# charles-kmc/Semi-blind-image-deblurring-problems-with-TV

Hardware: AMD Instinct MI355X
Metric: SALSA outer-iters/sec + final PSNR, 2048x2048 Gaussian blur (higher is better)
Workload: dtype f64; 1 GPU; SALSA_v2 TV deblur, one 2048x2048 image per GPU, Gaussian PSF 7x7, BSNR 30 dB, TViters=10; images_per_gpu=1, parallelism=images x1

## Files before the change

include/sbtv.h:

```cpp
#ifndef SBTV_H
#define SBTV_H

#include <stddef.h>

#ifdef __cplusplus
extern "C" {
#endif

#define SBTV_VERSION 100

#define SBTV_HOST_PTRS   0
#define SBTV_DEVICE_PTRS 1
#define SBTV_REDUCE_DEVICE  2
#define SBTV_SAPG_HOST_LOOP 4
#define SBTV_FISTA_EXACT_PROX 2

#define SBTV_OK                   0
#define SBTV_ERR_BADARG          -1
#define SBTV_ERR_SIZE            -2
#define SBTV_ERR_MAXITER         -3
#define SBTV_ERR_DUALVARS        -4
#define SBTV_ERR_MODE            -5
#define SBTV_ERR_STOPCRITERION   -6
#define SBTV_ERR_INIT            -7
// ... 200 lines not shown
                       int chambolleit, unsigned long long seed, int chain_offset, const double *noise,
                       double *x_out, const sbtv_moments_opts *mo, double *post_mean, double *post_var,
                       long long *post_count, int flags);

typedef struct sbtv_myula_wavelet_opts {
    int    samples;
    double lambda, gamma;
    unsigned long long seed;
    int    chain_offset;
} sbtv_myula_wavelet_opts;
int sbtv_myula_wavelet(sbtv_ctx *ctx, const double *y, int M, int N, int batch,
                       const double *taps, int taille, const double *h, int hlen, int levels,
                       const sbtv_myula_wavelet_opts *op,
                       const double *theta, const double *sigma2,
                       const double *xw0, const double *noise,
                       double *gx, double *logpi,
                       double *xw_last,
                       const sbtv_moments_opts *mo,
                       double *post_mean, double *post_var, long long *post_count,
                       double *coef_mean, double *coef_var,
                       int flags);

int sbtv_max_eigenval(sbtv_ctx *ctx, const double *taps, int taille, const double *x0,
                      int M, int N, double tol, int max_iter, double *val, int *iters, int flags);

int sbtv_PSNR(sbtv_ctx *ctx, const double *x_true, const double *x, int M, int N, int batch, double *out, int flags);
int sbtv_MSE(sbtv_ctx *ctx, const double *x_true, const double *x, int M, int N, int batch, double *out, int flags);

typedef struct sbtv_group sbtv_group;
int         sbtv_group_create(const int *devices, int n, sbtv_group **out);
int         sbtv_group_destroy(sbtv_group *g);
int         sbtv_group_size(const sbtv_group *g);
sbtv_ctx   *sbtv_group_ctx(sbtv_group *g, int i);
const char *sbtv_group_last_error(const sbtv_group *g);
int         sbtv_group_shard_of(const sbtv_group *g, int n_items, int item, int *shard, int *first, int *count);
int sbtv_SALSA_v2_sharded(sbtv_group *g, const double *y, int M, int N, int n_items,
                          const double *taps, int taille, const double *tau, const double *mu,
                          const sbtv_salsa_opts *opts, const double *true_x, const double *x_init,
                          double *x_out, double *objective, double *distance, double *times, double *mses,
                          int *numA, int *numAt, int *n_outer);
int sbtv_SALSA_v2_sharded_dev(sbtv_group *g, const double *const *y, int M, int N, int n_items,
                              const double *taps, int taille, const double *tau, const double *mu,
                              const sbtv_salsa_opts *opts, const double *const *true_x,
                              const double *const *x_init, double *const *x_out, double *objective,
                              double *distance, double *times, double *mses, int *numA, int *numAt, int *n_outer);
int sbtv_SAPG_algorithm_sharded(sbtv_group *g, const double *y, int M, int N, int n_items,
                                const sbtv_sapg_opts *op, const double *x0, const double *noise,
                                double *thetas, double *ps, double *sigmas, double *logpi,
                                double *logpi_wu, double *gx, double *grads, double *eb, double *x_last);
int sbtv_fista_tv_sharded(sbtv_group *g, const double *b, int M, int N, int n_items,
                          const double *taps, int taille, const double *tau, double L,
                          int prox_iters, int stopcriterion, double tolerance, int maxiters,
                          int zero_start, const double *true_x, double *x_out,
                          double *objective, double *mses, int *n_iter);
int sbtv_CSALSA_v2_sharded(sbtv_group *g, const double *y, int M, int N, int n_items,
                           const double *taps, int taille, const double *mu1, const double *mu2,
                           const double *sigma, const double *epsilon, double continuationfactor,
                           const sbtv_salsa_opts *opts, const double *true_x, const double *x_init,
                           double *x_out, double *objective, double *distance1, double *distance2,
                           double *criterion, double *times, double *mses,
                           int *numA, int *numAt, int *n_outer);
int sbtv_CoRAL_v2_sharded(sbtv_group *g, const double *y, int M, int N, int n_items,
                          const double *taps, int taille, const double *tau1, const double *tau2,
                          const double *mu1, const double *mu2, const double *mu_ls, int TViters2,
                          const sbtv_salsa_opts *opts, const double *true_x, const double *x_init,
                          double *x_out, double *objective, double *distance, double *times, double *mses,
                          int *numA, int *numAt, int *n_outer);
int sbtv_SALSA_masked_sharded(sbtv_group *g, const double *y, const double *mask, int M, int N, int n_items,
                              const double *taps, int taille, const double *tau, const double *mu1, const double *mu2,
                              const sbtv_salsa_opts *opts, const double *true_x, const double *x_init,
                              double *x_out, double *objective, double *distance, double *times, double *mses,
                              int *numA, int *numAt, int *n_outer);

int sbtv_host_transpose(const double *src, double *dst, int batch, int rows, int cols);
int sbtv_diag_solve_stats(const sbtv_ctx *ctx, double out[4]);
int sbtv_diag_stage_stats(const sbtv_ctx *ctx, double out[4]);
int sbtv_diag_canary(sbtv_ctx *ctx, int poke, int *enabled, int *nbuf, int *nbad);
int sbtv_last_host_stats(const sbtv_ctx *ctx, double out[14]);
int sbtv_diag_workspace(sbtv_ctx *ctx, const char *name, void **dptr, size_t *bytes);
int sbtv_diag_switches(char *buf, size_t cap);
int sbtv_diag_time_pass(sbtv_ctx *ctx, int pass, int M, int N, int batch, int reps, double *ms_avg, double *alg_bytes);
int sbtv_diag_prox_variant(sbtv_ctx *ctx, int M, int N, int batch, int out[6]);
int sbtv_diag_prox_geometry(sbtv_ctx *ctx, int M, int N, int batch, int out[16]);
int sbtv_diag_fft_plan(sbtv_ctx *ctx, int M, int N, int batch, int out[16]);
typedef struct sbtv_diag_pass {
    int M, N, batch, op, epilogue, taille, shared_spec, repeats;
    const double *x, *add;
    const double *taps, *d1taps, *d2taps;
    const double *y, *e0;
    const double *mu, *cs;
    const int *frozen;
    const double *u, *bu_in, *tru, *xprev, *sub_b;
    double alpha;
    double *bu, *ystep;
    double *x_out, *g_out, *acc, *sums, *tv;
} sbtv_diag_pass;
int sbtv_diag_spectral_pass(sbtv_ctx *ctx, const sbtv_diag_pass *args);

#ifdef __cplusplus
}
#endif
#endif
```

semi-blind-image-deblurring-problems-with-tv_amd/csrc/admm.hip:

```cpp
#include <chrono>
#include <cmath>

#include "sbtv_internal.h"

#pragma clang fp contract(off)

namespace sbtv {

namespace {

constexpr int AB = 256;

__device__ __forceinline__ double ad_wave_sum(double v) {
#pragma unroll
    for (int off = 32; off > 0; off >>= 1) v += __shfl_xor(v, off, 64);
    return v;
}

template <int NQ>
__device__ __forceinline__ void ad_store_partials(double (&acc)[NQ], double *__restrict__ partials) {
    __shared__ double red[NQ * 4];
    const int lane = threadIdx.x & 63, w = threadIdx.x >> 6;
#pragma unroll
    for (int c = 0; c < NQ; ++c) {
// ... 350 lines not shown
    double2 *S, *Hs, *Ys;
    double *taps_d;
    double inv_scale, parseval;
    bool spectral = false;
};

int admm_common(sbtv_ctx *ctx, int M, int N, const double *taps, int taille, const double *yd, AdmmCommon *c) {
    if (((size_t)M * N) & 1)
        return fail(ctx, SBTV_ERR_SIZE, "this entry point needs an even number of pixels (its element-wise passes move two per lane)");
    SBTV_TRY(fft_plan(ctx, M, N, 1, &c->fp));
    c->P = (size_t)M * N;
    SBTV_TRY(ws_get_t(ctx, "admm.S", c->fp.s_img, &c->S));
    SBTV_TRY(ws_get_t(ctx, "admm.H", c->fp.u_img, &c->Hs));
    SBTV_TRY(ws_get_t(ctx, "admm.Y", c->fp.u_img, &c->Ys));
    SBTV_TRY(ws_get_t(ctx, "admm.taps", (size_t)taille * taille, &c->taps_d));
    SBTV_HIP(ctx, hipMemcpyAsync(c->taps_d, taps, sizeof(double) * taille * taille, hipMemcpyHostToDevice, ctx->stream));
    SBTV_HIP(ctx, hipStreamSynchronize(ctx->stream));
    c->inv_scale = 1.0 / ((double)c->fp.n1 * N);
    c->parseval = 1.0 / ((double)M * N);
    SBTV_TRY(psf_spectrum(ctx, c->fp, c->taps_d, taille, c->Hs));
    if (yd) {
        RowsArgs a{};
        a.dir_fwd = 1;
        a.op = OP_NONE;
        SBTV_TRY(fft_cols_fwd(ctx, c->fp, yd, nullptr, c->S));
        SBTV_TRY(fft_rows(ctx, c->fp, c->S, c->S, a));
        SBTV_TRY(spec_unpack(ctx, c->fp, c->S, c->Ys));
    }
    return 0;
}

int admm_apply(sbtv_ctx *ctx, const AdmmCommon &c, int op, const double *in, double *out) {
    RowsArgs a{};
    a.dir_fwd = 1;
    a.dir_inv = 1;
    a.op = op;
    a.H = c.Hs;
    SBTV_TRY(fft_cols_fwd(ctx, c.fp, in, nullptr, c.S));
    SBTV_TRY(fft_rows(ctx, c.fp, c.S, c.S, a));
    return fft_cols_inv(ctx, c.fp, c.S, out, c.inv_scale);
}

int admm_init_x(sbtv_ctx *ctx, const AdmmCommon &c, int initialization, const double *yd, const double *xi, double *x) {
    if (initialization == 0) {
        SBTV_HIP(ctx, hipMemsetAsync(x, 0, sizeof(double) * c.P, ctx->stream));
    } else if (initialization == 2) {
        SBTV_TRY(admm_apply(ctx, c, OP_MUL_HC, yd, x));
    } else {
        SBTV_HIP(ctx, hipMemcpyAsync(x, xi, sizeof(double) * c.P, hipMemcpyDeviceToDevice, ctx->stream));
    }
    return 0;
}

int check_common(sbtv_ctx *ctx, const char *who, const double *y, const double *taps, const sbtv_salsa_opts *opts,
                 const double *x_init, int M, int N, int batch, int taille) {
    if (!y || !opts || batch < 1) return fail(ctx, SBTV_ERR_BADARG, std::string(who) + ": missing required argument");
    if (!taps) return fail(ctx, SBTV_ERR_MISSING_AT, "The function handle for transpose of A is missing");
    if (opts->stopcriterion < 1 || opts->stopcriterion > 3) return fail(ctx, SBTV_ERR_STOPCRITERION, "Unknown stopping criterion");
    if (opts->initialization != 0 && opts->initialization != 2 && opts->initialization != 33333)
        return fail(ctx, SBTV_ERR_INIT, "Unknown 'Initialization' option");
    if (opts->initialization == 33333 && !x_init) return fail(ctx, SBTV_ERR_INIT, "Initialization = array but x_init is NULL");
    if (opts->TViters <= 0) return fail(ctx, SBTV_ERR_MAXITER, std::string(who) + ": TViters must be positive");
    if (opts->maxiter < 1) return fail(ctx, SBTV_ERR_MAXITER, std::string(who) + ": maxiter must be positive");
    if (taille < 1 || taille > 15 || taille > M || taille > N) return fail(ctx, SBTV_ERR_PSF, "Mask does not fit inside array");
    return 0;
}

inline bool csalsa_spectral_wanted() {
    static const bool on = [] {
        const char *e = getenv("SBTV_CSALSA_SPECTRAL");
        return !(e && e[0] == '0');
    }();
    return on;
}

inline int admm_prox(sbtv_ctx *ctx, const ProxPlan &pp, const double *g, int K, double *f, bool spec, long long *nlaunch,
                     double *stepsums, const double *lam_dev, double tol, double tau) {
    if (!spec) {
        SBTV_TRY(prox_reset(ctx, pp, lam_dev, 1.0, K, tol, tau, true, nullptr));
        return prox_iterate(ctx, pp, g, K, f);
    }
    SBTV_TRY(prox_iterate(ctx, pp, g, K, f, false, 1, (int)(*nlaunch & 1), nullptr));
    *nlaunch += prox_launches(pp, K);
    return reduce_partials(ctx, pp.partials, K, pp.fnblk, stepsums);
}

struct AdmmSlots {
    hipEvent_t ev[2] = {nullptr, nullptr};
    ~AdmmSlots() {
        for (auto e : ev)
            if (e) (void)hipEventDestroy(e);
    }
};

int csalsa_one(sbtv_ctx *ctx, const double *yd, int M, int N, const double *taps, int taille, double mu1, double mu2,
               double sigma, double epsilon, double delta, const sbtv_salsa_opts *opts, const double *td,
               const double *xi, double *x_out_dev, double *objective, double *distance1, double *distance2,
               double *criterion, double *times, double *mses, int *numA, int *numAt, int *n_outer, bool spec_wanted) {
    AdmmCommon c;
    {
        FftPlan chk;
        SBTV_TRY(fft_plan(ctx, M, N, 1, &chk));
        const bool sp = delta == 1.0 && csalsa_spectral_wanted() && fft_rows_csalsa_ok(chk) && !(M & 1) &&
                        (size_t)M * N < ((size_t)1 << 31);
        SBTV_TRY(admm_common(ctx, M, N, taps, taille, sp ? yd : nullptr, &c));
        c.spectral = sp;
    }
    const bool spectral = c.spectral;
    ProxPlan pp;
    SBTV_TRY(prox_plan(ctx, M, N, 1, &pp));
    const size_t P = c.P;
    const int nb = ad_blocks(P);
    double *xbuf[2], *u, *bu, *v, *bv, *w, *Ax, *g, *par, *partials, *sums, *acc;
    double2 *Ws;
    SBTV_TRY(ws_get_t(ctx, "admm.acc", (size_t)3 * fft_rows_blocks(c.fp), &acc));
    SBTV_TRY(ws_get_t(ctx, "admm.x0", P, &xbuf[0]));
    SBTV_TRY(ws_get_t(ctx, "admm.x1", P, &xbuf[1]));
    SBTV_TRY(ws_get_t(ctx, "admm.u", P, &u));
    SBTV_TRY(ws_get_t(ctx, "admm.bu", P, &bu));
    SBTV_TRY(ws_get_t(ctx, "admm.v", P, &v));
    SBTV_TRY(ws_get_t(ctx, "admm.bv", P, &bv));
    SBTV_TRY(ws_get_t(ctx, "admm.w", P, &w));
    SBTV_TRY(ws_get_t(ctx, "admm.Ax", P, &Ax));
    SBTV_TRY(ws_get_t(ctx, "admm.g", P, &g));
    SBTV_TRY(ws_get_t(ctx, "admm.par", (size_t)4, &par));
    SBTV_TRY(ws_get_t(ctx, "admm.partials", (size_t)8 * nb, &partials));
    SBTV_TRY(ws_get_t(ctx, "admm.sums", (size_t)64, &sums));
    SBTV_TRY(ws_get_t(ctx, "admm.W", c.fp.u_img, &Ws));
    double2 *Es = Ws;
    double *cst = nullptr, *rs = nullptr;
    SBTV_TRY(ws_get_t(ctx, "admm.cs", (size_t)8, &cst));
    SBTV_TRY(ws_get_t(ctx, "admm.rs", (size_t)4, &rs));
    double *hs = nullptr;
    {
        void *pz = nullptr;
        SBTV_TRY(pinned_get(ctx, sizeof(double) * 128, &pz));
        hs = static_cast<double *>(pz);
    }
    const int maxiter = opts->maxiter;
    if (!(epsilon != 0.0)) epsilon = sqrt((double)P + 8 * sqrt((double)P)) * sigma;
    auto upload_par = [&]() -> int {
        const double h[4] = {mu1, mu2, 1.0 / mu1, 0.0};
        SBTV_HIP(ctx, hipMemcpyAsync(par, h, sizeof(h), hipMemcpyHostToDevice, ctx->stream));
        SBTV_HIP(ctx, hipStreamSynchronize(ctx->stream));
        return 0;
    };
    SBTV_TRY(upload_par());
    int h_numA = 0, h_numAt = 1;
    ctx->calls += 2;
    double *x = xbuf[0];
    SBTV_TRY(admm_init_x(ctx, c, opts->initialization, yd, xi, x));
    if (opts->initialization == 0) ctx->calls += 1;
    if (opts->initialization == 2) h_numAt += 1;
    SBTV_HIP(ctx, hipMemsetAsync(u, 0, sizeof(double) * P, ctx->stream));
    SBTV_HIP(ctx, hipMemsetAsync(bu, 0, sizeof(double) * P, ctx->stream));
    SBTV_HIP(ctx, hipMemsetAsync(v, 0, sizeof(double) * P, ctx->stream));
    SBTV_HIP(ctx, hipMemsetAsync(bv, 0, sizeof(double) * P, ctx->stream));
    SBTV_TRY(prox_zero_duals(ctx, pp));
    SBTV_TRY(prox_reset(ctx, pp, par + 2, 1.0, opts->TViters, opts->chambolle_tol, opts->chambolle_tau, false, nullptr));

    SBTV_TRY(admm_apply(ctx, c, OP_MUL_H, x, Ax));
    h_numA += 2;
    ctx->calls += 2;
    {
        double *sv, *sbv, *sbu;
        SBTV_TRY(ws_get_t(ctx, "admm.scratch0", P, &sv));
        SBTV_TRY(ws_get_t(ctx, "admm.scratch1", P, &sbv));
        SBTV_TRY(ws_get_t(ctx, "admm.scratch2", P, &sbu));
        SBTV_HIP(ctx, hipMemsetAsync(sbv, 0, sizeof(double) * P, ctx->stream));
        SBTV_HIP(ctx, hipMemsetAsync(sbu, 0, sizeof(double) * P, ctx->stream));
        SBTV_HIP(ctx, hipMemsetAsync(sums, 0, sizeof(double) * 16, ctx->stream));
        hipLaunchKernelGGL(csalsa_update_kernel, dim3(nb), dim3(AB), 0, ctx->stream, Ax, yd, x, u, sv, sbv, sbu, td,
                           (const double *)nullptr, sums + 8, 1.0, partials, P);
        SBTV_TRY(reduce_partials(ctx, partials, 6, nb, sums));
        SBTV_TRY(tvnorm_dev(ctx, x, M, N, 1, sums + 6));
        SBTV_HIP(ctx, hipMemcpyAsync(hs, sums, sizeof(double) * 8, hipMemcpyDeviceToHost, ctx->stream));
        SBTV_HIP(ctx, hipStreamSynchronize(ctx->stream));
        if (criterion) criterion[0] = sqrt(hs[0]);
        if (distance1) distance1[0] = sqrt(hs[0]);
        if (distance2) distance2[0] = sqrt(hs[2]);
        if (objective) objective[0] = hs[6];
        if (mses && td) mses[0] = hs[3] / (double)P;
        if (times) times[0] = 0.0;
    }
    double crit_prev = sqrt(hs[0]), obj_prev = hs[6];
    const auto t0 = std::chrono::steady_clock::now();
    SBTV_HIP(ctx, hipEventRecord(ctx->ev[0], ctx->stream));
    const int K = opts->TViters;
    const bool spec = spec_wanted && delta == 1.0 && prox_spec_ok(pp, g, u, K);
    const int lag = (spec && (opts->speculate & 1)) ? 1 : 0;
    long long nlaunch = 0, prox_iters = 0;
    AdmmSlots slots;
    for (auto &e : slots.ev) SBTV_HIP(ctx, hipEventCreateWithFlags(&e, hipEventDisableTiming));
    double *hslot[2] = {hs, hs + 64};
    const bool tv_fused = fft_cols_tv_ok(c.fp);
    const int ntv = tv_fused ? fft_cols_blocks(c.fp) : 0;
    double *tvp = nullptr;
    if (tv_fused) SBTV_TRY(ws_get_t(ctx, "admm.tvc", (size_t)ntv, &tvp));
    if (spectral) {
        const double h[8] = {mu2, mu2, 0.0, 0.0, 0.0, 0.0, 0.0, 0.0};
        SBTV_HIP(ctx, hipMemsetAsync(Es, 0, sizeof(double2) * c.fp.u_img, ctx->stream));
        SBTV_HIP(ctx, hipMemcpyAsync(cst, h, sizeof(h), hipMemcpyHostToDevice, ctx->stream));
        SBTV_HIP(ctx, hipStreamSynchronize(ctx->stream));
    }
    auto enqueue_spectral = [&](int outer) -> int {
        const int k = outer - 1;
        double *xn = xbuf[k & 1];
        const double *xprev = xbuf[(k & 1) ^ 1];
        RowsArgs a{};
        a.dir_fwd = 1;
        a.dir_inv = 1;
        a.op = OP_CSALSA;
        a.H = c.Hs;
        a.Y = c.Ys;
        a.E = Es;
        a.cs = cst;
        a.mu = par;
        a.acc = acc;
        SBTV_TRY(fft_cols_fwd(ctx, c.fp, u, bu, c.S));
        SBTV_TRY(fft_rows(ctx, c.fp, c.S, c.S, a));
        if (fft_cols_inv_step_ok(c.fp)) {
            SBTV_TRY(fft_cols_inv_sub(ctx, c.fp, c.S, xn, c.inv_scale, bu, g));
        } else {
            SBTV_TRY(fft_cols_inv(ctx, c.fp, c.S, xn, c.inv_scale));
            hipLaunchKernelGGL(ad_sub_kernel, dim3(nb), dim3(AB), 0, ctx->stream, xn, bu, g, P);
        }
        hipLaunchKernelGGL(csalsa_scal_kernel, dim3(1), dim3(256), 0, ctx->stream, acc, fft_rows_blocks(c.fp), cst, epsilon,
                           c.parseval, sums);
        RedJobs jb;
        if (!spec) {
            SBTV_TRY(admm_prox(ctx, pp, g, K, u, false, &nlaunch, sums + 16, par + 2, opts->chambolle_tol, opts->chambolle_tau));
        } else {
            SBTV_TRY(prox_iterate(ctx, pp, g, K, u, false, 1, (int)(nlaunch & 1), nullptr));
            nlaunch += prox_launches(pp, K);
            jb.add(pp.partials, K, pp.fnblk, sums + 16);
        }
        hipLaunchKernelGGL(csalsa_post_kernel, dim3(nb), dim3(AB), 0, ctx->stream, xn, u, bu, td,
                           (opts->stopcriterion == 2) ? xprev : (const double *)nullptr, partials, (unsigned)M, (unsigned)N, P);
        jb.add(partials, 5, nb, sums + 2);
        SBTV_TRY(reduce_jobs(ctx, jb));
        SBTV_HIP(ctx, hipGetLastError());
        double *hsl = hslot[outer & 1];
        SBTV_HIP(ctx, hipMemcpyAsync(hsl, sums, sizeof(double) * (16 + (spec ? K : 0)), hipMemcpyDeviceToHost, ctx->stream));
        if (!spec) SBTV_HIP(ctx, hipMemcpyAsync(hsl + 8, pp.ctrl, sizeof(int), hipMemcpyDeviceToHost, ctx->stream));
        SBTV_HIP(ctx, hipEventRecord(slots.ev[outer & 1], ctx->stream));
        return 0;
    };
    auto enqueue = [&](int outer) -> int {
        if (spectral) return enqueue_spectral(outer);
        const int k = outer - 1;
        double *xn = xbuf[k & 1];
        const double *xprev = xbuf[(k & 1) ^ 1];
        hipLaunchKernelGGL(csalsa_w_kernel, dim3(nb), dim3(AB), 0, ctx->stream, yd, v, bv, par, w, P);
        {
            RowsArgs a{};
            a.dir_fwd = 1;
            a.op = OP_NONE;
            SBTV_TRY(fft_cols_fwd(ctx, c.fp, w, nullptr, c.S));
            SBTV_TRY(fft_rows(ctx, c.fp, c.S, c.S, a));
            SBTV_TRY(spec_unpack(ctx, c.fp, c.S, Ws));
        }
        {
            RowsArgs a{};
            a.dir_fwd = 1;
            a.dir_inv = 1;
            a.op = OP_SALSA;
            a.H = c.Hs;
            a.Y = Ws;
            a.mu = par;
            a.acc = acc;
            SBTV_TRY(fft_cols_fwd(ctx, c.fp, u, bu, c.S));
            SBTV_TRY(fft_rows(ctx, c.fp, c.S, c.S, a));
            SBTV_TRY(fft_cols_inv(ctx, c.fp, c.S, xn, c.inv_scale));
        }
        hipLaunchKernelGGL(ad_sub_kernel, dim3(nb), dim3(AB), 0, ctx->stream, xn, bu, g, P);
        SBTV_TRY(admm_prox(ctx, pp, g, K, u, spec, &nlaunch, sums + 16, par + 2, opts->chambolle_tol, opts->chambolle_tau));
        {
            RowsArgs a{};
            a.dir_fwd = 1;
            a.dir_inv = 1;
            a.op = OP_MUL_H;
            a.H = c.Hs;
            SBTV_TRY(fft_cols_fwd_f(ctx, c.fp, xn, nullptr, c.S, nullptr, tvp));
            SBTV_TRY(fft_rows(ctx, c.fp, c.S, c.S, a));
            SBTV_TRY(fft_cols_inv(ctx, c.fp, c.S, Ax, c.inv_scale));
        }
        hipLaunchKernelGGL(csalsa_ve_kernel, dim3(nb), dim3(AB), 0, ctx->stream, Ax, yd, bv, partials, P);
        SBTV_TRY(reduce_partials(ctx, partials, 1, nb, sums + 8));
        hipLaunchKernelGGL(csalsa_update_kernel, dim3(nb), dim3(AB), 0, ctx->stream, Ax, yd, xn, u, v, bv, bu, td,
                           (opts->stopcriterion == 2) ? xprev : (const double *)nullptr, sums + 8, epsilon, partials, P);
        SBTV_TRY(reduce_partials(ctx, partials, 6, nb, sums));
        if (tv_fused) SBTV_TRY(reduce_partials(ctx, tvp, 1, ntv, sums + 6));
        else SBTV_TRY(tvnorm_dev(ctx, xn, M, N, 1, sums + 6));
        SBTV_HIP(ctx, hipGetLastError());
        double *hsl = hslot[outer & 1];
        SBTV_HIP(ctx, hipMemcpyAsync(hsl, sums, sizeof(double) * (16 + (spec ? K : 0)), hipMemcpyDeviceToHost, ctx->stream));
        if (!spec) SBTV_HIP(ctx, hipMemcpyAsync(hsl + 8, pp.ctrl, sizeof(int), hipMemcpyDeviceToHost, ctx->stream));
        SBTV_HIP(ctx, hipEventRecord(slots.ev[outer & 1], ctx->stream));
        return 0;
    };
    bool stop = false;
    auto process = [&](int outer) -> int {
        const int k = outer - 1;
        const double *hsl = hslot[outer & 1];
        SBTV_HIP(ctx, hipEventSynchronize(slots.ev[outer & 1]));
        if (spec) SBTV_TRY(spec_stop_rule(ctx, pp, hsl + 16, K, opts->chambolle_tol));
        prox_iters += spec ? K : *reinterpret_cast<const int *>(hsl + 8);
        h_numAt += 1;
        h_numA += 1;
        ctx->calls += 3;
        const double crit = sqrt(hsl[0]), obj = hsl[6];
        if (criterion) criterion[k] = crit;
        if (distance1) distance1[k] = sqrt(hsl[1]);
        if (distance2) distance2[k] = sqrt(hsl[2]);
        if (objective) objective[k] = obj;
        if (mses && td) mses[k] = hsl[3] / (double)P;
        if (times) times[k] = std::chrono::duration<double>(std::chrono::steady_clock::now() - t0).count();
        if (delta != 1.0) {
// ... 62 lines not shown
    {
        void *pz = nullptr;
        SBTV_TRY(pinned_get(ctx, sizeof(double) * 192, &pz));
        hs = static_cast<double *>(pz);
    }
    {
        const double h[4] = {mu_ls, tau1 / mu1, tau2 / mu2, 0.0};
        SBTV_HIP(ctx, hipMemcpyAsync(par, h, sizeof(h), hipMemcpyHostToDevice, ctx->stream));
        SBTV_HIP(ctx, hipStreamSynchronize(ctx->stream));
    }
    const int maxiter = opts->maxiter;
    int h_numA = 0, h_numAt = 2;
    ctx->calls += 3;
    double *x = xbuf[0];
    SBTV_TRY(admm_init_x(ctx, c, opts->initialization, yd, xi, x));
    if (opts->initialization == 0) ctx->calls += 1;
    for (double *dst : {u, bu, v, bv})
        SBTV_HIP(ctx, hipMemcpyAsync(dst, x, sizeof(double) * P, hipMemcpyDeviceToDevice, ctx->stream));
    SBTV_HIP(ctx, hipMemsetAsync(g1, 0, sizeof(double) * P, ctx->stream));
    SBTV_HIP(ctx, hipMemsetAsync(g2, 0, sizeof(double) * P, ctx->stream));
    SBTV_TRY(prox_zero_duals(ctx, pu));
    SBTV_TRY(prox_reset(ctx, pu, par + 1, 1.0, opts->TViters, opts->chambolle_tol, opts->chambolle_tau, false, nullptr));
    if (!batched) {
        SBTV_TRY(prox_zero_duals(ctx, pv));
        SBTV_TRY(prox_reset(ctx, pv, par + 2, 1.0, TViters2, opts->chambolle_tol, opts->chambolle_tau, false, nullptr));
    }

    {
        RowsArgs a{};
        a.dir_fwd = 1;
        a.op = OP_RESID;
        a.H = c.Hs;
        a.Y = c.Ys;
        a.acc = acc;
        SBTV_TRY(fft_cols_fwd(ctx, c.fp, x, nullptr, c.S));
        SBTV_TRY(fft_rows(ctx, c.fp, c.S, nullptr, a));
        SBTV_TRY(reduce_partials(ctx, acc, 1, nrb, sums + 8));
        SBTV_TRY(tvnorm_dev(ctx, u, M, N, 1, sums + 9));
        SBTV_HIP(ctx, hipMemsetAsync(sums, 0, sizeof(double) * 8, ctx->stream));
        if (td) {
            double *o4 = nullptr;
            SBTV_TRY(ws_get_t(ctx, "admm.o4", (size_t)4, &o4));
            SBTV_TRY(pair_sums(ctx, x, td, P, 1, o4));
            SBTV_HIP(ctx, hipMemcpyAsync(sums, o4, sizeof(double), hipMemcpyDeviceToDevice, ctx->stream));
        }
        SBTV_HIP(ctx, hipMemcpyAsync(hs, sums, sizeof(double) * 16, hipMemcpyDeviceToHost, ctx->stream));
        SBTV_HIP(ctx, hipStreamSynchronize(ctx->stream));
        h_numA += 1;
        ctx->calls += 1;
        const double f0 = 0.5 * (hs[8] * c.parseval) + tau1 * hs[9] + tau2 * hs[9];
        if (objective) objective[0] = f0;
        if (times) times[0] = 0.0;
        if (mses && td) mses[0] = hs[0] / (double)P;
        hs[15] = f0;
    }
    double obj_prev = hs[15];
    const auto t0 = std::chrono::steady_clock::now();
    SBTV_HIP(ctx, hipEventRecord(ctx->ev[0], ctx->stream));
    const int K1 = opts->TViters, K2 = TViters2;
    const bool spec = spec_wanted && prox_spec_ok(pu, g1, u, K1) &&
                      (batched || prox_spec_ok(pv, g2, v, K2));
    const int lag = (spec && (opts->speculate & 1)) ? 1 : 0;
    long long nl_u = 0, nl_v = 0, prox_iters = 0;
    AdmmSlots slots;
    for (auto &e : slots.ev) SBTV_HIP(ctx, hipEventCreateWithFlags(&e, hipEventDisableTiming));
    double *hslot[2] = {hs, hs + 96};
    auto enqueue = [&](int outer) -> int {
        double *xn = xbuf[outer & 1];
        const double *xprev = xbuf[(outer & 1) ^ 1];
        const bool sp = spec && outer >= 2;
        RedJobs jb;
        if (spec && outer == 2) {
            SBTV_TRY(prox_reset(ctx, pu, par + 1, 1.0, K1, opts->chambolle_tol, opts->chambolle_tau, true, nullptr));
            if (!batched) SBTV_TRY(prox_reset(ctx, pv, par + 2, 1.0, K2, opts->chambolle_tol, opts->chambolle_tau, true, nullptr));
        }
        if (batched) {
            static_assert(FSTRIDE == 32, "the step sums of the second prox are read at sums + 48");
            if (!sp) {
                SBTV_TRY(prox_reset(ctx, pu, par + 1, 1.0, K1, opts->chambolle_tol, opts->chambolle_tau, true, nullptr));
                SBTV_TRY(prox_iterate(ctx, pu, g1, K1, u));
            } else {
                SBTV_TRY(prox_iterate(ctx, pu, g1, K1, u, false, 1, (int)(nl_u & 1), nullptr));
                nl_u += prox_launches(pu, K1);
                jb.add(pu.partials, FSTRIDE + K1, pu.fnblk, sums + 16);
            }
        } else {
            SBTV_TRY(admm_prox(ctx, pu, g1, K1, u, sp, &nl_u, sums + 16, par + 1, opts->chambolle_tol, opts->chambolle_tau));
            SBTV_TRY(admm_prox(ctx, pv, g2, K2, v, sp, &nl_v, sums + 48, par + 2, opts->chambolle_tol, opts->chambolle_tau));
        }
        if (tv_in_s) {
            hipLaunchKernelGGL(coral_s_kernel<true>, dim3(nb), dim3(AB), 0, ctx->stream, u, bu, v, bv, mu1, mu2, mu_ls, s, tvpart,
                               (unsigned)M, (unsigned)N, P);
            jb.add(tvpart, 2, nb, sums + 9);
        } else {
            hipLaunchKernelGGL(coral_s_kernel<false>, dim3(nb), dim3(AB), 0, ctx->stream, u, bu, v, bv, mu1, mu2, mu_ls, s, tvpart,
                               (unsigned)M, (unsigned)N, P);
        }
        {
            RowsArgs a{};
            a.dir_fwd = 1;
            a.dir_inv = 1;
            a.op = OP_SALSA;
            a.H = c.Hs;
            a.Y = c.Ys;
            a.mu = par;
            a.acc = acc;
            SBTV_TRY(fft_cols_fwd(ctx, c.fp, s, nullptr, c.S));
            SBTV_TRY(fft_rows(ctx, c.fp, c.S, c.S, a));
            SBTV_TRY(fft_cols_inv(ctx, c.fp, c.S, xn, c.inv_scale));
        }
        hipLaunchKernelGGL(coral_post_kernel, dim3(nb), dim3(AB), 0, ctx->stream, xn,
                           (opts->stopcriterion == 2) ? xprev : (const double *)nullptr, u, v, bu, bv, g1, g2, td, partials, P);
        jb.add(partials, 7, nb, sums);
        jb.add(acc, 1, nrb, sums + 8);
        SBTV_TRY(reduce_jobs(ctx, jb));
        if (!tv_in_s) {
            SBTV_TRY(tvnorm_dev(ctx, u, M, N, 1, sums + 9));
            SBTV_TRY(tvnorm_dev(ctx, v, M, N, 1, sums + 10));
        }
        SBTV_HIP(ctx, hipGetLastError());
        double *hsl = hslot[outer & 1];
        SBTV_HIP(ctx, hipMemcpyAsync(hsl, sums, sizeof(double) * (sp ? 80 : 12), hipMemcpyDeviceToHost, ctx->stream));
        if (!sp) {
            SBTV_HIP(ctx, hipMemcpyAsync(hsl + 12, pu.ctrl, sizeof(int), hipMemcpyDeviceToHost, ctx->stream));
            SBTV_HIP(ctx, hipMemcpyAsync(hsl + 13, batched ? pu.ctrl + 1 : pv.ctrl, sizeof(int), hipMemcpyDeviceToHost, ctx->stream));
        }
        SBTV_HIP(ctx, hipEventRecord(slots.ev[outer & 1], ctx->stream));
        return 0;
    };
    bool stop = false;
    auto process = [&](int outer) -> int {
        const double *hsl = hslot[outer & 1];
        const bool sp = spec && outer >= 2;
        SBTV_HIP(ctx, hipEventSynchronize(slots.ev[outer & 1]));
        if (sp) {
            SBTV_TRY(spec_stop_rule(ctx, pu, hsl + 16, K1, opts->chambolle_tol));
            if (!batched) SBTV_TRY(spec_stop_rule(ctx, pv, hsl + 48, K2, opts->chambolle_tol));
        }
        prox_iters += sp ? (long long)(K1 + K2)
                         : (long long)(*reinterpret_cast<const int *>(hsl + 12) + *reinterpret_cast<const int *>(hsl + 13));
        h_numA += 1;
        ctx->calls += 2;
        const double f = 0.5 * (hsl[8] * c.parseval) + tau1 * hsl[9] + tau2 * hsl[10];
        if (objective) objective[outer] = f;
        if (mses && td) mses[outer] = hsl[0] / (double)P;
        if (distance) {
            distance[(size_t)(outer - 1) * 2] = sqrt(hsl[1]) / sqrt(hsl[3] + hsl[4]);
            distance[(size_t)(outer - 1) * 2 + 1] = sqrt(hsl[2]) / sqrt(hsl[3] + hsl[5]);
        }
        if (times) times[outer] = std::chrono::duration<double>(std::chrono::steady_clock::now() - t0).count();
        if (outer > 1) {
            double crit;
            if (opts->stopcriterion == 1)
                crit = fabs(f - obj_prev) / obj_prev;
            else if (opts->stopcriterion == 2)
                crit = fabs(sqrt(hsl[6]) / sqrt(hsl[3]));
            else
                crit = f;
            stop = crit < opts->tolA;
        }
        obj_prev = f;
        return 0;
    };
    int last = 0;
    SBTV_TRY(pipelined_loop(ctx, &last, maxiter, lag, false, enqueue, process, [&] { return !stop; }));
    SBTV_HIP(ctx, hipEventRecord(ctx->ev[1], ctx->stream));
    SBTV_HIP(ctx, hipStreamSynchronize(ctx->stream));
// ... 30 lines not shown
    SBTV_TRY(ws_get_t(ctx, "admm.g", P, &g));
    SBTV_TRY(ws_get_t(ctx, "admm.par", (size_t)4, &par));
    SBTV_TRY(ws_get_t(ctx, "admm.partials", (size_t)12 * nb, &partials));
    SBTV_TRY(ws_get_t(ctx, "admm.sums", (size_t)96, &sums));
    SBTV_TRY(ws_get_t(ctx, "admm.acc", (size_t)3 * nrb, &acc));
    SBTV_TRY(ws_get_t(ctx, "admm.W", c.fp.u_img, &Ws));
    SBTV_TRY(ws_get_t(ctx, "admm.S2", c.fp.s_img, &S2));
    double *hs = nullptr;
    {
        void *pz = nullptr;
        SBTV_TRY(pinned_get(ctx, sizeof(double) * 192, &pz));
        hs = static_cast<double *>(pz);
    }
    {
        const double h[4] = {mu1 / mu2, tau / mu1, 0.0, 0.0};
        SBTV_HIP(ctx, hipMemcpyAsync(par, h, sizeof(h), hipMemcpyHostToDevice, ctx->stream));
        SBTV_HIP(ctx, hipStreamSynchronize(ctx->stream));
    }
    const double bx_scale = c.fp.generic ? c.inv_scale : c.inv_scale / (double)N;
    auto post = [&](const double *xn, const double *xprev) {
        if (tv_in_post)
            hipLaunchKernelGGL(masked_post_kernel<true>, dim3(nb), dim3(AB), 0, ctx->stream, xn, xprev, (const double *)Bx,
                               (const double *)u, yd, md, bu, v, bv, g, td, mu2, partials, (unsigned)M, (unsigned)N, P);
        else
            hipLaunchKernelGGL(masked_post_kernel<false>, dim3(nb), dim3(AB), 0, ctx->stream, xn, xprev, (const double *)Bx,
                               (const double *)u, yd, md, bu, v, bv, g, td, mu2, partials, (unsigned)M, (unsigned)N, P);
    };
    const int maxiter = opts->maxiter;
    int h_numA = 0, h_numAt = 0;
    double *x = xbuf[0];
    if (opts->initialization == 2) {
        hipLaunchKernelGGL(masked_my_kernel, dim3(nb), dim3(AB), 0, ctx->stream, md, yd, g, P);
        SBTV_TRY(admm_apply(ctx, c, OP_MUL_HC, g, x));
        h_numAt += 1;
        ctx->calls += 1;
    } else {
        SBTV_TRY(admm_init_x(ctx, c, opts->initialization, yd, xi, x));
    }
    SBTV_TRY(admm_apply(ctx, c, OP_MUL_H, x, Bx));
    h_numA += 1;
    ctx->calls += 1;
    SBTV_HIP(ctx, hipMemcpyAsync(u, x, sizeof(double) * P, hipMemcpyDeviceToDevice, ctx->stream));
    SBTV_HIP(ctx, hipMemcpyAsync(v, Bx, sizeof(double) * P, hipMemcpyDeviceToDevice, ctx->stream));
    SBTV_HIP(ctx, hipMemsetAsync(bu, 0, sizeof(double) * P, ctx->stream));
    SBTV_HIP(ctx, hipMemsetAsync(bv, 0, sizeof(double) * P, ctx->stream));
    SBTV_TRY(prox_zero_duals(ctx, pp));
    SBTV_TRY(prox_reset(ctx, pp, par + 1, 1.0, opts->TViters, opts->chambolle_tol, opts->chambolle_tau, false, nullptr));
    {
        SBTV_HIP(ctx, hipMemsetAsync(sums, 0, sizeof(double) * 16, ctx->stream));
        post(x, nullptr);
        SBTV_TRY(reduce_partials(ctx, partials, nq, nb, sums));
        if (!tv_in_post) SBTV_TRY(tvnorm_dev(ctx, u, M, N, 1, sums + 9));
        SBTV_HIP(ctx, hipGetLastError());
        SBTV_HIP(ctx, hipMemcpyAsync(hs, sums, sizeof(double) * 16, hipMemcpyDeviceToHost, ctx->stream));
        SBTV_HIP(ctx, hipStreamSynchronize(ctx->stream));
        const double f0 = 0.5 * hs[0] + tau * hs[9];
        if (objective) objective[0] = f0;
        if (times) times[0] = 0.0;
        if (mses && td) mses[0] = hs[7] / (double)P;
        hs[15] = f0;
    }
    double obj_prev = hs[15];
    const auto t0 = std::chrono::steady_clock::now();
    SBTV_HIP(ctx, hipEventRecord(ctx->ev[0], ctx->stream));
    const int K = opts->TViters;
    const bool spec = spec_wanted && prox_spec_ok(pp, g, u, K);
    const int lag = (spec && (opts->speculate & 1)) ? 1 : 0;
    long long nlaunch = 0, prox_iters = 0;
    AdmmSlots slots;
    for (auto &e : slots.ev) SBTV_HIP(ctx, hipEventCreateWithFlags(&e, hipEventDisableTiming));
    double *hslot[2] = {hs, hs + 96};
    auto enqueue = [&](int outer) -> int {
        double *xn = xbuf[outer & 1];
        const double *xprev = xbuf[(outer & 1) ^ 1];
        const bool sp = spec && outer >= 2;
        RedJobs jb;
        if (spec && outer == 2)
            SBTV_TRY(prox_reset(ctx, pp, par + 1, 1.0, K, opts->chambolle_tol, opts->chambolle_tau, true, nullptr));
        if (!sp) {
            SBTV_TRY(admm_prox(ctx, pp, g, K, u, false, &nlaunch, sums + 16, par + 1, opts->chambolle_tol, opts->chambolle_tau));
        } else {
            SBTV_TRY(prox_iterate(ctx, pp, g, K, u, false, 1, (int)(nlaunch & 1), nullptr));
            nlaunch += prox_launches(pp, K);
            jb.add(pp.partials, K, pp.fnblk, sums + 16);
        }
        {
            RowsArgs a{};
            a.dir_fwd = 1;
            a.op = OP_NONE;
            SBTV_TRY(fft_cols_fwd(ctx, c.fp, v, bv, S2));
            SBTV_TRY(fft_rows(ctx, c.fp, S2, S2, a));
            SBTV_TRY(spec_unpack(ctx, c.fp, S2, Ws));
        }
        {
            RowsArgs a{};
            a.dir_fwd = 1;
            a.dir_inv = 1;
            a.op = OP_SALSA;
            a.H = c.Hs;
            a.Y = Ws;
            a.mu = par;
            a.acc = acc;
            SBTV_TRY(fft_cols_fwd(ctx, c.fp, u, bu, c.S));
            SBTV_TRY(fft_rows(ctx, c.fp, c.S, c.S, a));
            SBTV_TRY(fft_cols_inv(ctx, c.fp, c.S, xn, c.inv_scale));
        }
        {
            RowsArgs a{};
            a.dir_fwd = 1;
            a.dir_inv = 1;
            a.op = OP_MUL_H;
            a.H = c.Hs;
            SBTV_TRY(fft_rows(ctx, c.fp, c.S, S2, a));
            SBTV_TRY(fft_cols_inv(ctx, c.fp, S2, Bx, bx_scale));
        }
        post(xn, (opts->stopcriterion == 2) ? xprev : (const double *)nullptr);
        jb.add(partials, nq, nb, sums);
        SBTV_TRY(reduce_jobs(ctx, jb));
        if (!tv_in_post) SBTV_TRY(tvnorm_dev(ctx, u, M, N, 1, sums + 9));
        SBTV_HIP(ctx, hipGetLastError());
        double *hsl = hslot[outer & 1];
        SBTV_HIP(ctx, hipMemcpyAsync(hsl, sums, sizeof(double) * (sp ? 16 + K : 12), hipMemcpyDeviceToHost, ctx->stream));
        if (!sp) SBTV_HIP(ctx, hipMemcpyAsync(hsl + 12, pp.ctrl, sizeof(int), hipMemcpyDeviceToHost, ctx->stream));
        SBTV_HIP(ctx, hipEventRecord(slots.ev[outer & 1], ctx->stream));
        return 0;
    };
    bool stop = false;
    auto process = [&](int outer) -> int {
        const double *hsl = hslot[outer & 1];
        const bool sp = spec && outer >= 2;
        SBTV_HIP(ctx, hipEventSynchronize(slots.ev[outer & 1]));
        if (sp) SBTV_TRY(spec_stop_rule(ctx, pp, hsl + 16, K, opts->chambolle_tol));
        prox_iters += sp ? (long long)K : (long long)*reinterpret_cast<const int *>(hsl + 12);
        h_numA += 1;
        h_numAt += 1;
        ctx->calls += 2;
        const double f = 0.5 * hsl[0] + tau * hsl[9];
        if (objective) objective[outer] = f;
        if (mses && td) mses[outer] = hsl[7] / (double)P;
        if (distance) {
            distance[(size_t)(outer - 1) * 2] = sqrt(hsl[1]) / sqrt(hsl[3] + hsl[4]);
            distance[(size_t)(outer - 1) * 2 + 1] = sqrt(hsl[2]) / sqrt(hsl[5] + hsl[6]);
        }
        if (times) times[outer] = std::chrono::duration<double>(std::chrono::steady_clock::now() - t0).count();
        if (outer > 1) {
            double crit;
            if (opts->stopcriterion == 1)
                crit = fabs(f - obj_prev) / obj_prev;
            else if (opts->stopcriterion == 2)
                crit = fabs(sqrt(hsl[8]) / sqrt(hsl[3]));
            else
                crit = f;
            stop = crit < opts->tolA;
        }
        obj_prev = f;
        return 0;
    };
    int last = 0;
    SBTV_TRY(pipelined_loop(ctx, &last, maxiter, lag, false, enqueue, process, [&] { return !stop; }));
    SBTV_HIP(ctx, hipEventRecord(ctx->ev[1], ctx->stream));
    SBTV_HIP(ctx, hipStreamSynchronize(ctx->stream));
    SBTV_TRY(loop_timing(ctx, 0.0, prox_iters, 1, P));
    SBTV_HIP(ctx, hipMemcpyAsync(x_out_dev, xbuf[last & 1], sizeof(double) * P, hipMemcpyDeviceToDevice, ctx->stream));
    SBTV_HIP(ctx, hipStreamSynchronize(ctx->stream));
    if (numA) *numA = h_numA;
    if (numAt) *numAt = h_numAt;
    if (n_outer) *n_outer = last;
// ... 346 lines not shown
```

semi-blind-image-deblurring-problems-with-tv_amd/csrc/ctx.hip:

```cpp
#include <chrono>
#include <cmath>
#include <cstring>
#include <algorithm>
#include <mutex>
#include <thread>
#include <vector>

#include "sbtv_internal.h"

namespace sbtv {

static std::string g_error;
static std::mutex g_error_mu;

void set_global_error(const std::string &msg) {
    std::lock_guard<std::mutex> lk(g_error_mu);
    g_error = msg;
}

int fail(sbtv_ctx *ctx, int code, const std::string &msg) {
    if (ctx) ctx->err = msg;
    set_global_error(msg);
    return code;
}
// ... 418 lines not shown
    ctx->calls = 0;
    return 0;
}

int sbtv_last_timing(const sbtv_ctx *ctx, double out[4]) {
    if (!ctx || !out) return SBTV_ERR_BADARG;
    for (int i = 0; i < 4; ++i) out[i] = ctx->timing[i];
    return 0;
}

int sbtv_last_host_stats(const sbtv_ctx *ctx, double out[14]) {
    if (!ctx || !out) return SBTV_ERR_BADARG;
    const HostStats &h = ctx->hstat;
    const double v[14] = {h.waits, h.ready_at_once, h.waits_slept, h.sleeps, h.stream_queries,
                          h.wait_s, h.wait_max_s, h.enqueue_s, h.enqueue_max_s, h.wait_max_outer,
                          h.nvcsw, h.nivcsw, h.minflt, h.majflt};
    for (int i = 0; i < 14; ++i) out[i] = v[i];
    return 0;
}

int sbtv_host_transpose(const double *src, double *dst, int batch, int rows, int cols) {
    if (!src || !dst || batch < 0 || rows < 0 || cols < 0) return SBTV_ERR_BADARG;
    constexpr int BS = 64;
    const long long nbr = ((long long)rows + BS - 1) / BS;
    const long long jobs = nbr * batch;
    auto work = [&](int t, int T) {
        for (long long job = t; job < jobs; job += T) {
            const int b = (int)(job / nbr), r0 = (int)(job % nbr) * BS, r1 = std::min(rows, r0 + BS);
            const double *s = src + (size_t)b * rows * cols;
            double *d = dst + (size_t)b * rows * cols;
            for (int c0 = 0; c0 < cols; c0 += BS) {
                const int c1 = std::min(cols, c0 + BS);
                for (int c = c0; c < c1; ++c)
                    for (int r = r0; r < r1; ++r) d[(size_t)c * rows + r] = s[(size_t)r * cols + c];
            }
        }
    };
    const size_t bytes = (size_t)batch * rows * cols * sizeof(double);
    const int T = bytes >= ((size_t)4 << 20) ? 4 : 1;
    std::vector<std::thread> th;
    int started = 1;
    try {
        for (int t = 1; t < T; ++t, ++started) th.emplace_back(work, t, T);
    } catch (...) {
    }
    work(0, T);
    for (auto &x : th) x.join();
    for (int t = started; t < T; ++t) work(t, T);
    return 0;
}

int sbtv_diag_solve_stats(const sbtv_ctx *ctx, double out[4]) {
    if (!ctx || !out) return SBTV_ERR_BADARG;
    for (int i = 0; i < 4; ++i) out[i] = ctx->solve_stats[i];
    if (ctx->lanes)
        for (int r = 0; r < sbtv_group_size(ctx->lanes); ++r)
            for (int i = 0; i < 4; ++i) out[i] += sbtv_group_ctx(ctx->lanes, r)->solve_stats[i];
    return 0;
}

int sbtv_diag_stage_stats(const sbtv_ctx *ctx, double out[4]) {
    if (!ctx || !out) return SBTV_ERR_BADARG;
    for (int i = 0; i < 4; ++i) out[i] = ctx->stage_stats[i];
    if (ctx->lanes)
        for (int r = 0; r < sbtv_group_size(ctx->lanes); ++r)
            for (int i = 0; i < 4; ++i) out[i] += sbtv_group_ctx(ctx->lanes, r)->stage_stats[i];
    return 0;
}

int sbtv_diag_workspace(sbtv_ctx *ctx, const char *name, void **dptr, size_t *bytes) {
    if (!ctx || !name || !dptr) return SBTV_ERR_BADARG;
    auto it = ctx->ws.find(name);
    if (it == ctx->ws.end() || !it->second.p) return fail(ctx, SBTV_ERR_BADARG, std::string("no workspace named '") + name + "'");
    *dptr = it->second.p;
    if (bytes) *bytes = it->second.bytes;
    return 0;
}

int sbtv_diag_switches(char *buf, size_t cap) {
    static const char *const names[] = {
        "SBTV_CANARY", "SBTV_COLLECT_RIDE", "SBTV_EXACT", "SBTV_FFT_WAVE", "SBTV_FISTA_FUSED_STEP", "SBTV_FISTA_LAG",
        "SBTV_FUSED_VARIANT", "SBTV_GRAPH", "SBTV_INLINE_CTRL", "SBTV_PROX_SPEC", "SBTV_SAPG_DEFER",
        "SBTV_SAPG_FUSED_MYULA", "SBTV_SAPG_HOST", "SBTV_SINGLE_STEP", "SBTV_SPIN", "SBTV_TAG_SPIN_US", "SBTV_TILE_ORDER", "SBTV_SALSA_NOX", "SBTV_CSALSA_SPECTRAL",
        "SBTV_CORAL_BATCH", "SBTV_ROWS_FOLD", "SBTV_ERR_SUBSET", "SBTV_LANES", "SBTV_LANE_COUNT", "SBTV_STAGE_THREADS", "SBTV_TEST_FAIL_SAPG", "SBTV_FUSED_STAGGER"};
    if (!buf || cap == 0) return SBTV_ERR_BADARG;
    std::string s;
    int nset = 0;
    for (const char *n : names)
        if (const char *e = getenv(n)) {
            s += (nset++ ? " " : "");
            s += n;
            s += "=";
            s += e;
        }
    if (s.size() + 1 > cap) s.resize(cap - 1);
    memcpy(buf, s.c_str(), s.size() + 1);
    return nset;
}

int sbtv_diag_canary(sbtv_ctx *ctx, int poke, int *enabled, int *nbuf, int *nbad) {
    if (!ctx) return SBTV_ERR_BADARG;
    SBTV_HIP(ctx, hipSetDevice(ctx->device));
    if (enabled) *enabled = ctx->canary ? 1 : 0;
    int nb = 0, bad = 0;
    if (ctx->canary && poke) {
        for (auto &kv : ctx->ws)
            if (kv.second.base) {
                SBTV_HIP(ctx, hipMemsetAsync(static_cast<unsigned char *>(kv.second.p) + kv.second.bytes, 0, 8, ctx->stream));
                break;
            }
    }
    std::string name;
    SBTV_TRY(canary_verify(ctx, &nb, &bad, &name));
    if (ctx->canary && poke && bad) {
        for (auto &kv : ctx->ws)
            if (kv.second.base) {
                SBTV_HIP(ctx, hipMemsetAsync(static_cast<unsigned char *>(kv.second.p) + kv.second.bytes, kGuardByte, kGuard, ctx->stream));
                break;
            }
        SBTV_HIP(ctx, hipStreamSynchronize(ctx->stream));
    }
    if (nbuf) *nbuf = nb;
    if (nbad) *nbad = bad;
    return 0;
}

int sbtv_malloc(sbtv_ctx *ctx, size_t bytes, void **dptr) {
    if (!ctx || !dptr) return SBTV_ERR_BADARG;
    SBTV_HIP(ctx, hipSetDevice(ctx->device));
    SBTV_HIP(ctx, hipMalloc(dptr, bytes));
    return 0;
}

int sbtv_free(sbtv_ctx *ctx, void *dptr) {
    if (!ctx) return SBTV_ERR_BADARG;
    SBTV_HIP(ctx, hipStreamSynchronize(ctx->stream));
    SBTV_HIP(ctx, hipFree(dptr));
    return 0;
}

int sbtv_memcpy_h2d(sbtv_ctx *ctx, void *dst, const void *src, size_t bytes) {
    if (!ctx) return SBTV_ERR_BADARG;
    SBTV_HIP(ctx, hipSetDevice(ctx->device));
    if (stage_threaded(bytes)) {
        SBTV_HIP(ctx, hipStreamSynchronize(ctx->stream));
        return stage_copy(ctx, dst, src, bytes, true);
    }
    SBTV_HIP(ctx, hipMemcpyAsync(dst, src, bytes, hipMemcpyHostToDevice, ctx->stream));
    SBTV_HIP(ctx, hipStreamSynchronize(ctx->stream));
    return 0;
}

int sbtv_memcpy_d2h(sbtv_ctx *ctx, void *dst, const void *src, size_t bytes) {
    if (!ctx) return SBTV_ERR_BADARG;
    SBTV_HIP(ctx, hipSetDevice(ctx->device));
    if (stage_threaded(bytes)) {
        SBTV_HIP(ctx, hipStreamSynchronize(ctx->stream));
        return stage_copy(ctx, dst, src, bytes, false);
    }
    SBTV_HIP(ctx, hipMemcpyAsync(dst, src, bytes, hipMemcpyDeviceToHost, ctx->stream));
    SBTV_HIP(ctx, hipStreamSynchronize(ctx->stream));
    return 0;
}

static double spectral_norm_sq(const double *D, int t) {
    double B[15 * 15];
    for (int i = 0; i < t; ++i)
// ... 78 lines not shown
```

semi-blind-image-deblurring-problems-with-tv_amd/csrc/fista.hip:

```cpp
#include <cmath>
#include <cstring>

#include "sbtv_internal.h"

namespace sbtv {

__global__ __launch_bounds__(256) void scale_kernel(double *__restrict__ x, double a, size_t n2) {
    for (size_t q = (size_t)blockIdx.x * 256 + threadIdx.x; q < n2; q += (size_t)gridDim.x * 256) {
        double2 v = reinterpret_cast<double2 *>(x)[q];
        v.x *= a;
        v.y *= a;
        reinterpret_cast<double2 *>(x)[q] = v;
    }
}

static int launch_scale(sbtv_ctx *ctx, double *x, double a, size_t n) {
    hipLaunchKernelGGL(scale_kernel, dim3(ew_blocks(n)), dim3(256), 0, ctx->stream, x, a, n / 2);
    SBTV_HIP(ctx, hipGetLastError());
    return 0;
}

__global__ __launch_bounds__(256) void fista_collect_kernel(const double *__restrict__ acc, int nrb,
                                                            const double *__restrict__ mom, int npb,
                                                            const double *__restrict__ tvp, int ntv,
// ... 97 lines not shown
        init_val = val;
        SBTV_TRY(launch_scale(ctx, x, 1.0 / val, P));
    }
    *val_out = val;
    if (iters) *iters = (k > max_iter) ? max_iter : k;
    return canary_epilogue(ctx, 0);
}

}

static int fista_solve(sbtv_ctx *ctx, const double *bd, int M, int N, int batch, const double *taps, int taille,
                       const double *tau, double L, int prox_iters, int stopcriterion, double tolerance, int maxiters,
                       int zero_start, const double *td, double *x_out, double *objective, double *mses, int *n_iter,
                       int flags, bool spec_wanted) {
    FftPlan fp;
    SBTV_TRY(fft_plan(ctx, M, N, batch, &fp));
    ProxPlan pp;
    SBTV_TRY(prox_plan(ctx, M, N, batch, &pp));
    const size_t P = (size_t)M * N, cnt = P * batch;
    double *xb[2] = {nullptr, nullptr}, *y = nullptr, *grad = nullptr, *xfinal = nullptr;
    SBTV_TRY(ws_get_t(ctx, "fista.x", cnt, &xb[1]));
    SBTV_TRY(ws_get_t(ctx, "fista.x2", cnt, &xb[0]));
    double *x = xb[1];
    SBTV_TRY(ws_get_t(ctx, "fista.y", cnt, &y));
    SBTV_TRY(ws_get_t(ctx, "fista.grad", cnt, &grad));
    SBTV_TRY(stage_out_buf(ctx, "fista.xfinal", x_out, cnt, flags, &xfinal));
    double2 *S = nullptr, *Hs = nullptr, *Bs = nullptr;
    SBTV_TRY(ws_get_t(ctx, "fista.S", (size_t)batch * fp.s_img, &S));
    SBTV_TRY(ws_get_t(ctx, "fista.H", (size_t)batch * fp.u_img, &Hs));
    SBTV_TRY(ws_get_t(ctx, "fista.B", (size_t)batch * fp.u_img, &Bs));
    const size_t npar = (size_t)batch * taille * taille + 2 * (size_t)batch;
    double *par = nullptr;
    SBTV_TRY(ws_get_t(ctx, "fista.par", npar, &par));
    double *taps_d = par, *lam_d = par + (size_t)batch * taille * taille;
    std::vector<double> hpar(npar);
    for (size_t q = 0; q < (size_t)batch * taille * taille; ++q) hpar[q] = taps[q];
    for (int b = 0; b < batch; ++b) {
        hpar[(size_t)batch * taille * taille + b] = tau[b] / L;
        hpar[(size_t)batch * taille * taille + batch + b] = 0.0;
    }
    SBTV_HIP(ctx, hipMemcpyAsync(par, hpar.data(), sizeof(double) * npar, hipMemcpyHostToDevice, ctx->stream));
    int *frozen_d = nullptr;
    SBTV_TRY(ws_get_t(ctx, "fista.frozen", (size_t)batch, &frozen_d));
    SBTV_HIP(ctx, hipMemsetAsync(frozen_d, 0, sizeof(int) * batch, ctx->stream));
    const int nrb = fft_rows_blocks(fp), npb = ew_blocks(P);
    double *acc = nullptr, *momp = nullptr, *o4 = nullptr;
    SBTV_TRY(ws_get_t(ctx, "fista.acc", (size_t)batch * 3 * nrb, &acc));
    SBTV_TRY(ws_get_t(ctx, "fista.momp", (size_t)batch * 3 * npb, &momp));
    SBTV_TRY(ws_get_t(ctx, "fista.o4", (size_t)batch * 4, &o4));
    constexpr int FT = 8 + FSTRIDE;
    const size_t slot_n = (size_t)FT * batch;
    double *scal_base_h = nullptr, *scal_base_hd = nullptr;
    SBTV_TRY(pinned_get(ctx, sizeof(double) * 4 * slot_n + sizeof(int) * batch, &scal_base_h, &scal_base_hd));
    for (size_t i = 0; i < 2 * slot_n; ++i) scal_base_h[2 * slot_n + i] = 0.0;
    int *frozen_h = reinterpret_cast<int *>(scal_base_h + 4 * slot_n);
    for (int b = 0; b < batch; ++b) frozen_h[b] = 0;
    double *tags_base_h = scal_base_h + 2 * slot_n, *tags_base_hd = scal_base_hd + 2 * slot_n;
    const double inv_scale = 1.0 / ((double)fp.n1 * N), parseval = 1.0 / ((double)M * N);
    SBTV_TRY(psf_spectrum(ctx, fp, taps_d, taille, Hs));
    {
        RowsArgs a{};
        a.dir_fwd = 1;
        SBTV_TRY(fft_cols_fwd(ctx, fp, bd, nullptr, S));
        SBTV_TRY(fft_rows(ctx, fp, S, S, a));
        SBTV_TRY(spec_unpack(ctx, fp, S, Bs));
    }
    if (zero_start) {
        SBTV_HIP(ctx, hipMemsetAsync(x, 0, sizeof(double) * cnt, ctx->stream));
    } else {
        RowsArgs a{};
        a.dir_fwd = 1;
        a.dir_inv = 1;
        a.op = OP_MUL_HC;
        a.H = Hs;
        SBTV_TRY(fft_cols_fwd(ctx, fp, bd, nullptr, S));
        SBTV_TRY(fft_rows(ctx, fp, S, S, a));
        SBTV_TRY(fft_cols_inv(ctx, fp, S, x, inv_scale));
    }
    SBTV_HIP(ctx, hipMemcpyAsync(y, x, sizeof(double) * cnt, hipMemcpyDeviceToDevice, ctx->stream));

    const bool out_aliases_input = (flags & SBTV_DEVICE_PTRS) && (overlaps(bd, x_out, cnt) || overlaps(td, x_out, cnt));
    const bool prox_spec = spec_wanted && !out_aliases_input && prox_spec_ok(pp, y, x, prox_iters);
    bool prox_was_spec = false;
    auto objective_of_x = [&](const double *xk, int k, const int *frozen, const double *mom_partials) -> int {
        RowsArgs a{};
        a.dir_fwd = 1;
        a.op = OP_RESID;
        a.H = Hs;
        a.Y = Bs;
        a.acc = acc;
        a.frozen = frozen;
        double *tvp = nullptr;
        int ntv = 0;
        if (fft_cols_tv_ok(fp)) {
            ntv = fft_cols_blocks(fp);
            SBTV_TRY(ws_get_t(ctx, "fista.tvc", (size_t)batch * ntv, &tvp));
        }
        SBTV_TRY(fft_cols_fwd_f(ctx, fp, xk, nullptr, S, frozen, tvp));
        SBTV_TRY(fft_rows(ctx, fp, S, nullptr, a));
        if (!tvp) SBTV_TRY(tvnorm_partials(ctx, xk, M, N, batch, &tvp, &ntv));
        const int slot = k & 1;
        hipLaunchKernelGGL(fista_collect_kernel, dim3(prox_was_spec ? 7 + prox_iters : 7, batch), dim3(256), 0, ctx->stream,
                           (const double *)acc, nrb, mom_partials, npb, (const double *)tvp, ntv, scal_base_hd + slot * slot_n,
                           batch, (const double *)pp.partials, pp.fnblk,
                           (unsigned long long)(uintptr_t)(tags_base_hd + slot * slot_n), (double)k);
        SBTV_HIP(ctx, hipGetLastError());
        return 0;
    };
    std::vector<double> obj_prev(batch, 0.0);
    std::vector<int> frozen(batch, 0), h_niter(batch, 1);
    SBTV_TRY(objective_of_x(x, 1, nullptr, nullptr));
    SBTV_TRY(pair_sums(ctx, x, td, P, batch, o4));
    {
        std::vector<double> h4((size_t)batch * 4);
        SBTV_HIP(ctx, hipMemcpyAsync(h4.data(), o4, sizeof(double) * 4 * batch, hipMemcpyDeviceToHost, ctx->stream));
        SBTV_HIP(ctx, hipStreamSynchronize(ctx->stream));
        const double *sc = scal_base_h + slot_n;
        for (int b = 0; b < batch; ++b) {
            const double f0 = 0.5 * (sc[(size_t)b * 3] * parseval) + tau[b] * sc[6 * (size_t)batch + b];
            obj_prev[b] = f0;
            if (objective) objective[(size_t)b * maxiters] = f0;
            if (mses) mses[(size_t)b * maxiters] = h4[(size_t)b * 4] / (double)P;
        }
    }
    static const int lag = [] {
        const char *e = getenv("SBTV_FISTA_LAG");
        return (e && e[0] == '0') ? 0 : 1;
    }();
    double t_enq = 1.0;
    int active = batch;
    bool slot_spec[2] = {false, false};
    static const bool fused_wanted = [] {
        const char *e = getenv("SBTV_FISTA_FUSED_STEP");
        return !(e && e[0] == '0');
    }();
    const bool fused_step = fused_wanted && prox_spec && fft_cols_inv_step_ok(fp);
    if (fused_step) SBTV_TRY(prox_reset(ctx, pp, lam_d, 1.0, prox_iters, CHAMBOLLE_TOL, CHAMBOLLE_TAU, false, frozen_d));
    auto enqueue = [&](int k) -> int {
        const double t_old = t_enq;
        double *xk = xb[k & 1];
        {
            RowsArgs a{};
            a.dir_fwd = 1;
            a.dir_inv = 1;
            a.op = OP_GRADF;
            a.H = Hs;
            a.Y = Bs;
            a.acc = acc;
            a.frozen = frozen_d;
            SBTV_TRY(fft_cols_fwd_f(ctx, fp, y, nullptr, S, frozen_d));
            SBTV_TRY(fft_rows(ctx, fp, S, S, a));
            if (fused_step) {
                SBTV_TRY(fft_cols_inv_step(ctx, fp, S, y, inv_scale, 1.0 / L, frozen_d));
            } else {
                SBTV_TRY(fft_cols_inv_f(ctx, fp, S, grad, inv_scale, frozen_d));
                const ProxArm arm{pp.ctrl, lam_d, prox_iters, CHAMBOLLE_TOL, CHAMBOLLE_TAU, frozen_d};
                if (batch <= 256) {
                    SBTV_TRY(axpy(ctx, y, grad, 1.0 / L, cnt, &arm, batch));
                } else {
                    SBTV_TRY(axpy(ctx, y, grad, 1.0 / L, cnt));
                    SBTV_TRY(prox_reset(ctx, pp, lam_d, 1.0, prox_iters, CHAMBOLLE_TOL, CHAMBOLLE_TAU, false, frozen_d));
                }
            }
        }
        prox_was_spec = prox_spec;
        slot_spec[k & 1] = prox_spec;
        SBTV_TRY(prox_iterate(ctx, pp, y, prox_iters, xk, true, prox_spec));
        t_enq = 0.5 * (1 + sqrt(1 + 4 * t_old * t_old));
        SBTV_TRY(fista_momentum(ctx, xk, xb[(k - 1) & 1], y, td, (t_old - 1) / t_enq, momp, P, batch, frozen_d));
        SBTV_TRY(objective_of_x(xk, k, frozen_d, momp));
        return 0;
    };
    auto process = [&](int k) -> int {
        SBTV_TRY(wait_tags(ctx, tags_base_h + (size_t)(k & 1) * slot_n, batch, FT, 7, slot_spec[k & 1] ? prox_iters : 0,
                           (double)k));
        const double *sc = scal_base_h + (size_t)(k & 1) * slot_n;
        if (slot_spec[k & 1])
            SBTV_TRY(spec_stop_rule(ctx, pp, sc + 8 * (size_t)batch, prox_iters, CHAMBOLLE_TOL, frozen.data()));
        bool changed = false;
        for (int b = 0; b < batch; ++b) {
            if (frozen[b]) continue;
            const double f = 0.5 * (sc[(size_t)b * 3] * parseval) + tau[b] * sc[6 * (size_t)batch + b];
            const double *mom = sc + 3 * (size_t)batch + (size_t)b * 3;
            if (objective) objective[(size_t)b * maxiters + (k - 1)] = f;
            if (mses) mses[(size_t)b * maxiters + (k - 1)] = mom[0] / (double)P;
            h_niter[b] = k;
            double crit;
            if (stopcriterion == 1)
                crit = fabs(f - obj_prev[b]) / f;
            else if (stopcriterion == 2)
                crit = sqrt(mom[1]) / sqrt(mom[2]);
            else
                crit = f;
            obj_prev[b] = f;
            if (crit < tolerance) {
                frozen[b] = 1;
                frozen_h[b] = 1;
                --active;
                changed = true;
                SBTV_HIP(ctx, hipMemcpyAsync(xfinal + (size_t)b * P, xb[k & 1] + (size_t)b * P, sizeof(double) * P,
                                             hipMemcpyDeviceToDevice, ctx->stream));
            }
        }
        if (changed && active > 0) SBTV_TRY(upload_frozen(ctx, frozen_h, frozen_d, batch, fused_step ? pp.ctrl : nullptr));
        return 0;
    };
    int done = 1;
    SBTV_TRY(pipelined_loop(ctx, &done, maxiters, lag, true, enqueue, process, [&] { return active > 0; }));
    for (int b = 0; b < batch; ++b)
        if (!frozen[b])
            SBTV_HIP(ctx, hipMemcpyAsync(xfinal + (size_t)b * P, xb[h_niter[b] & 1] + (size_t)b * P, sizeof(double) * P,
                                         hipMemcpyDeviceToDevice, ctx->stream));
    SBTV_TRY(stage_out_copy(ctx, x_out, xfinal, cnt, flags));
    SBTV_HIP(ctx, hipStreamSynchronize(ctx->stream));
    if (n_iter)
        for (int b = 0; b < batch; ++b) n_iter[b] = h_niter[b];
    return 0;
}

int sbtv_fista_tv(sbtv_ctx *ctx, const double *bimg, int M, int N, int batch, const double *taps, int taille,
                  const double *tau, double L, int prox_iters, int stopcriterion, double tolerance, int maxiters,
                  int zero_start, const double *true_x, double *x_out, double *objective, double *mses, int *n_iter,
                  int flags) {
    if (!ctx) return SBTV_ERR_BADARG;
    if (!bimg || !taps || !tau || !true_x || batch < 1 || maxiters < 1 || !(L > 0.0))
        return fail(ctx, SBTV_ERR_BADARG, "fista_tv: bad arguments (b, taps, tau, true are required)");
    if (stopcriterion < 1 || stopcriterion > 3) return fail(ctx, SBTV_ERR_STOPCRITERION, "Invalid stopping criterion!");
    if (prox_iters <= 0) return fail(ctx, SBTV_ERR_MAXITER, "fista_tv: prox_iters must be positive");
    if (taille < 1 || taille > 15 || taille > M || taille > N) return fail(ctx, SBTV_ERR_PSF, "Mask does not fit inside array");
    SBTV_HIP(ctx, hipSetDevice(ctx->device));
    if (((size_t)M * N) & 1)
        return fail(ctx, SBTV_ERR_SIZE, "this entry point needs an even number of pixels (its element-wise passes move two per lane)");
    if (sbtv_group *lg = lanes_group(ctx, batch, false)) {
        LaneCall lc(ctx, lg);
        return lc.done(fista_sharded(lg, bimg, M, N, batch, taps, taille, tau, L, prox_iters, stopcriterion, tolerance, maxiters,
                                     zero_start, true_x, x_out, objective, mses, n_iter, flags), batch);
    }
    const size_t cnt = (size_t)M * N * batch;
    const double *bd = nullptr, *td = nullptr;
    SBTV_TRY(stage_in(ctx, "fista.b", bimg, cnt, flags, &bd));
    SBTV_TRY(stage_in(ctx, "fista.true", true_x, cnt, flags, &td));
    return canary_epilogue(ctx, solve_with_exact_repeat(ctx, !(flags & SBTV_FISTA_EXACT_PROX), [&](bool spec) {
        return fista_solve(ctx, bd, M, N, batch, taps, taille, tau, L, prox_iters, stopcriterion, tolerance, maxiters,
                           zero_start, td, x_out, objective, mses, n_iter, flags, spec);
    }));
}
```

semi-blind-image-deblurring-problems-with-tv_amd/csrc/salsa.hip:

```cpp
#include <algorithm>
#include <chrono>
#include <cmath>

#include <time.h>

#include "sbtv_internal.h"

namespace sbtv {

__global__ void salsa_setup_kernel(const double *__restrict__ src, double *__restrict__ par, int npar, int *__restrict__ frozen,
                                   int batch) {
    for (int i = threadIdx.x; i < npar; i += blockDim.x) par[i] = src[i];
    for (int b = threadIdx.x; b < batch; b += blockDim.x) frozen[b] = 0;
}

__global__ __launch_bounds__(256) void salsa_recover_x_kernel(const double *__restrict__ g, const double *__restrict__ bu,
                                                               double *__restrict__ x, size_t P) {
#pragma clang fp contract(off)
    for (size_t q = (size_t)blockIdx.x * 256 + threadIdx.x; q < P / 2; q += (size_t)gridDim.x * 256) {
        const double2 a = *reinterpret_cast<const double2 *>(g + 2 * q), b = *reinterpret_cast<const double2 *>(bu + 2 * q);
        *reinterpret_cast<double2 *>(x + 2 * q) = make_double2(a.x + b.x, a.y + b.y);
    }
}

// ... 150 lines not shown
    }
    SBTV_TRY(prox_reset(ctx, pp, thr_d, 1.0, opts->TViters, opts->chambolle_tol, opts->chambolle_tau, false, nullptr));

    std::vector<double> obj_prev(batch);
    double *o4 = nullptr;
    SBTV_TRY(ws_get_t(ctx, "salsa.o4", (size_t)batch * 4, &o4));
    {
        Collect c{};
        if (zero_init) {
            double *accz = nullptr, *postz = nullptr;
            int nz = 0;
            SBTV_TRY(salsa_zero_start(ctx, yd, want_mse ? td : nullptr, x, u, bu, P, batch, (double)M * (double)N, &accz, &postz,
                                      &nz));
            c = Collect{accz, nz, nullptr, 0, postz, nz, nullptr, 0, 0, 0ull, nullptr};
        } else {
            double *tvp = nullptr;
            int ntv = 0;
            RowsArgs a{};
            a.dir_fwd = 1;
            a.op = OP_RESID;
            a.H = Hs;
            a.Y = Ys;
            a.acc = acc;
            SBTV_TRY(fft_cols_fwd(ctx, fp, x, nullptr, S));
            SBTV_TRY(tvnorm_partials(ctx, u, M, N, batch, &tvp, &ntv));
            SBTV_TRY(fft_rows(ctx, fp, S, nullptr, a));
            if (want_mse) SBTV_TRY(pair_sums(ctx, x, td, P, batch, o4));
            c = Collect{acc, nrb, tvp, ntv, nullptr, 0, nullptr, 0, 0, 0ull, want_mse ? o4 : nullptr};
        }
        hipLaunchKernelGGL(salsa_collect_kernel, dim3(7, batch), dim3(256), 0, ctx->stream, c, (ProxCtrl *)nullptr,
                           (unsigned long long)(uintptr_t)init_hd, (const int *)nullptr, 0,
                           (unsigned long long)(uintptr_t)init_tags_hd, 1.0);
        SBTV_HIP(ctx, hipGetLastError());
        ctx->calls += batch;
    }
    bool init_read = false;
    auto read_initial = [&]() -> int {
        if (init_read) return 0;
        init_read = true;
        volatile const double *tg = init_tags_h;
        for (unsigned spin = 0;; ++spin) {
            bool ready = true;
            for (int b = 0; b < batch && ready; ++b)
                for (int i = 0; i < 8 && ready; ++i) ready = (tg[(size_t)b * SALSA_TAGS + i] == 1.0);
            if (ready) break;
            if (spin > 2000) {
                SBTV_HIP(ctx, hipStreamSynchronize(ctx->stream));
                break;
            }
            struct timespec ts = {0, 5000};
            nanosleep(&ts, nullptr);
        }
        __atomic_thread_fence(__ATOMIC_ACQUIRE);
        for (int b = 0; b < batch; ++b) {
            h_numA[b] += 1;
            const double f0 = 0.5 * (init_h[b].resid2 * parseval) + tau[b] * init_h[b].tv_u;
            obj_prev[b] = f0;
            if (objective) objective[(size_t)b * (maxiter + 1)] = f0;
            if (times) times[(size_t)b * (maxiter + 1)] = 0.0;
            if (mses && want_mse) mses[(size_t)b * (maxiter + 1)] = init_h[b].mse_num / (double)P;
        }
        return 0;
    };

    std::vector<int> frozen(batch, 0), h_nouter(batch, 0);
    int active = batch;
    double ms_prox = 0.0;
    long long prox_iters_run = 0;
    GraphExecs res;
    for (auto &e : ctx->loop_ev)
        if (!e) SBTV_HIP(ctx, hipEventCreate(&e));
    hipEvent_t ev_done[2] = {ctx->loop_ev[0], ctx->loop_ev[1]}, ev_p0[2] = {ctx->loop_ev[2], ctx->loop_ev[3]},
               ev_p1[2] = {ctx->loop_ev[4], ctx->loop_ev[5]};
    hipGraphExec_t(&gexec)[2] = res.g;
    const auto t0 = std::chrono::steady_clock::now();

    bool prox_timed[2] = {false, false};
    const bool spec_ok = spec_wanted && !graph_wanted(cnt) && prox_spec_ok(pp, g, u, opts->TViters);
    static const bool piggyback = [] {
        const char *e = getenv("SBTV_COLLECT_RIDE");
        return !(e && e[0] == '0');
    }();
    bool slot_tagged[2] = {false, false}, slot_spec[2] = {false, false};
    long long prox_iters_timed = 0;
    struct PendingCollect {
        bool valid = false;
        int outer = 0;
        bool spec = false;
    } pend;
    const int nl_prox = prox_launches(pp, opts->TViters);
    const bool zero_start = (opts->initialization == 0);
    auto make_collect = [&](int outer, bool spec) -> Collect {
        const int slot = outer & 1;
        return Collect{acc, nrb, nullptr, 0, postp, npb, spec ? pp.partials + (size_t)slot * pp.part_stride : nullptr, pp.fnblk,
                       opts->TViters, (unsigned long long)(uintptr_t)(psum_hd + (size_t)slot * batch * FSTRIDE), nullptr};
    };
    auto launch_collect = [&](int outer, bool spec, bool tagged) -> int {
        const int slot = outer & 1;
        const Collect c = make_collect(outer, spec);
        hipLaunchKernelGGL(salsa_collect_kernel, dim3(spec ? 7 + opts->TViters : 7, batch), dim3(256), 0, ctx->stream, c, pp.ctrl,
                           (unsigned long long)(uintptr_t)(scal_hd + (size_t)slot * batch), (const int *)frozen_d, 1,
                           tagged ? (unsigned long long)(uintptr_t)(tags_hd + (size_t)slot * batch * SALSA_TAGS) : 0ull, (double)outer);
        SBTV_HIP(ctx, hipGetLastError());
        return 0;
    };
    auto flush_pending = [&]() -> int {
        if (!pend.valid) return 0;
        pend.valid = false;
        return launch_collect(pend.outer, pend.spec, true);
    };
    auto enqueue_body = [&](int outer, bool eager) -> int {
        const int slot = outer & 1;
        const bool tagged = eager;
        const bool spec = spec_ok && outer >= 2;
        const bool timed = eager && ((outer & 31) == 4 || outer == 12);
        slot_tagged[slot] = tagged;
        slot_spec[slot] = spec;
        double *xn = (direct_last && outer == maxiter) ? x_out : xbuf[slot];
        const double *xprev = xbuf[slot ^ 1];
        SideJob side{};
        if (pend.valid && spec) {
            const int ps = pend.outer & 1;
            side.c = make_collect(pend.outer, pend.spec);
            side.out_addr = (unsigned long long)(uintptr_t)(scal_hd + (size_t)ps * batch);
            side.tags_addr = (unsigned long long)(uintptr_t)(tags_hd + (size_t)ps * batch * SALSA_TAGS);
            side.frozen = frozen_d;
            side.seq = (double)pend.outer;
            side.nblocks = 7 + (pend.spec ? opts->TViters : 0);
            pend.valid = false;
        } else {
            SBTV_TRY(flush_pending());
        }
        if (timed) SBTV_HIP(ctx, hipEventRecord(ev_p0[slot], ctx->stream));
        ProxPlan pps = pp;
        pps.partials = pp.partials + (size_t)slot * pp.part_stride;
        if (!(zero_start && outer == 1))
            SBTV_TRY(prox_iterate(ctx, pps, gb[(outer - 1) & 1], opts->TViters, u, outer == (zero_start ? 2 : 1), spec,
                                  spec ? ((outer - 2) * nl_prox) & 1 : 0, side.nblocks ? &side : nullptr));
        if (timed) SBTV_HIP(ctx, hipEventRecord(ev_p1[slot], ctx->stream));
        prox_timed[slot] = timed;
        RowsArgs a{};
        a.dir_fwd = 1;
        a.dir_inv = 1;
        a.op = OP_SALSA;
        a.H = Hs;
        a.Y = Ys;
        a.mu = mu_d;
        a.acc = acc;
        a.frozen = frozen_d;
        SBTV_TRY(fft_cols_fwd_f(ctx, fp, u, bub[(outer - 1) & 1], S, frozen_d));
        SBTV_TRY(fft_rows(ctx, fp, S, S, a));
        ColsPost cp;
        cp.u = u;
        cp.bu = bub[outer & 1];
        cp.g = gb[outer & 1];
        if (nox) {
            cp.bu_in = bub[(outer - 1) & 1];
            cp.skip_x = 1;
        }
        cp.tru = td;
        cp.xprev = crit2 ? xprev : nullptr;
        cp.partials = postp;
        SBTV_TRY(fft_cols_inv_post(ctx, fp, S, xn, inv_scale, frozen_d, cp));
        if (spec && eager && lag == 1 && outer < maxiter && piggyback) {
            pend.valid = true;
            pend.outer = outer;
            pend.spec = spec;
            return 0;
        }
        return launch_collect(outer, spec, tagged);
    };
    bool use_graph = graph_wanted(cnt);
    auto enqueue = [&](int outer) -> int {
        const int slot = outer & 1;
        if (use_graph && outer >= 3) {
            if (!gexec[slot]) {
                if (graph_begin(ctx) != 0 || graph_end(ctx, enqueue_body(outer, false), &gexec[slot]) != 0) {
                    use_graph = false;
                    gexec[slot] = nullptr;
                }
            }
            if (gexec[slot]) {
                SBTV_HIP(ctx, hipGraphLaunch(gexec[slot], ctx->stream));
                SBTV_HIP(ctx, hipEventRecord(ev_done[slot], ctx->stream));
                return 0;
            }
        }
        SBTV_TRY(enqueue_body(outer, true));
        return 0;
    };
    auto process = [&](int outer) -> int {
        const int slot = outer & 1;
        SBTV_TRY(read_initial());
        if (pend.valid && pend.outer == outer) SBTV_TRY(flush_pending());
        if (slot_tagged[slot])
            SBTV_TRY(wait_tags(ctx, tags_h + (size_t)slot * batch * SALSA_TAGS, batch, SALSA_TAGS, 8,
                               slot_spec[slot] ? opts->TViters : 0, (double)outer));
        else SBTV_TRY(wait_event(ctx, ev_done[slot]));
        if (prox_timed[slot]) {
            float ms = 0.f;
            SBTV_HIP(ctx, hipEventSynchronize(ev_p1[slot]));
            SBTV_HIP(ctx, hipEventElapsedTime(&ms, ev_p0[slot], ev_p1[slot]));
            ms_prox += ms;
            for (int b = 0; b < batch; ++b)
                if (!frozen[b]) prox_iters_timed += slot_spec[slot] ? (long long)opts->TViters : (long long)scal_h[(size_t)slot * batch + b].pad;
            prox_timed[slot] = false;
        }
        if (slot_spec[slot])
            SBTV_TRY(spec_stop_rule(ctx, pp, psum_h + (size_t)slot * batch * FSTRIDE, opts->TViters, opts->chambolle_tol,
                                    frozen.data()));
        const double tnow = std::chrono::duration<double>(std::chrono::steady_clock::now() - t0).count();
        bool changed = false;
        for (int b = 0; b < batch; ++b) {
            if (frozen[b]) continue;
            const SalsaScal &s = scal_h[(size_t)slot * batch + b];
            h_numA[b] += 1;
            h_nouter[b] = outer;
            double prox_k = s.pad;
// ... 108 lines not shown
```

semi-blind-image-deblurring-problems-with-tv_amd/csrc/sbtv_internal.h:

```cpp
#pragma once
#include <hip/hip_runtime.h>

#include <chrono>
#include <map>
#include <string>
#include <vector>

#include "../../include/sbtv.h"

namespace sbtv {

constexpr int kWave = 64;

struct ProxCtrl {
    int k;
    int done;
    int cur;
    int maxiter;
    int redo;
    int f_valid;
    double err;
    double lambda;
    double tol;
    double tau;
// ... 278 lines not shown
                 double *logpi_wu, double *gx, double *grads, double *eb, double *x_last, int flags,
                 const MomReq *mom = nullptr);
int sapg_impl(sbtv_ctx *ctx, const double *y, int M, int N, int batch, const sbtv_sapg_opts *op, const double *x0,
              const double *noise, double *thetas, double *ps, double *sigmas, double *logpi, double *logpi_wu, double *gx,
              double *grads, double *eb, double *x_last, sbtv_allreduce_fn reduce_fn, void *reduce_user, int flags,
              const MomReq *mom);
int fista_sharded(::sbtv_group *g, const double *b, int M, int N, int n_items, const double *taps, int taille,
                  const double *tau, double L, int prox_iters, int stopcriterion, double tolerance, int maxiters,
                  int zero_start, const double *true_x, double *x_out, double *objective, double *mses, int *n_iter,
                  int flags);
int csalsa_sharded(::sbtv_group *g, const double *y, int M, int N, int n_items, const double *taps, int taille,
                   const double *mu1, const double *mu2, const double *sigma, const double *epsilon,
                   double continuationfactor, const sbtv_salsa_opts *opts, const double *true_x, const double *x_init,
                   double *x_out, double *objective, double *distance1, double *distance2, double *criterion,
                   double *times, double *mses, int *numA, int *numAt, int *n_outer, int flags);
int coral_sharded(::sbtv_group *g, const double *y, int M, int N, int n_items, const double *taps, int taille,
                  const double *tau1, const double *tau2, const double *mu1, const double *mu2, const double *mu_ls,
                  int TViters2, const sbtv_salsa_opts *opts, const double *true_x, const double *x_init, double *x_out,
                  double *objective, double *distance, double *times, double *mses, int *numA, int *numAt, int *n_outer,
                  int flags);
int masked_sharded(::sbtv_group *g, const double *y, const double *mask, int M, int N, int n_items, const double *taps,
                   int taille, const double *tau, const double *mu1, const double *mu2, const sbtv_salsa_opts *opts,
                   const double *true_x, const double *x_init, double *x_out, double *objective, double *distance,
                   double *times, double *mses, int *numA, int *numAt, int *n_outer, int flags);

int wait_event(sbtv_ctx *ctx, hipEvent_t ev);
int wait_stream(sbtv_ctx *ctx);
int wait_tags(sbtv_ctx *ctx, const double *tags, int batch, int stride, int nscal, int nstep, double seq);

bool graph_wanted(size_t total_px);
int graph_begin(sbtv_ctx *ctx);
int graph_end(sbtv_ctx *ctx, int body_rc, hipGraphExec_t *exec);
struct GraphExecs {
    hipGraphExec_t g[2] = {nullptr, nullptr};
    ~GraphExecs() {
        for (auto e : g)
            if (e) (void)hipGraphExecDestroy(e);
    }
};

int loop_timing(sbtv_ctx *ctx, double prox_ms, long long prox_iters, int batch, size_t P);
void host_stats_begin(sbtv_ctx *ctx);
void host_stats_end(sbtv_ctx *ctx);

template <class Enqueue, class Process, class Active>
int pipelined_loop(sbtv_ctx *ctx, int *done, int maxiter, int lag, bool stats, Enqueue &&enqueue, Process &&process,
                   Active &&active) {
    if (stats) host_stats_begin(ctx);
    int rc = 0, enq = *done;
    while (rc == 0 && active() && *done < maxiter) {
        while (rc == 0 && enq < maxiter && enq - *done <= lag) {
            const auto te = std::chrono::steady_clock::now();
            rc = enqueue(++enq);
            const double d = std::chrono::duration<double>(std::chrono::steady_clock::now() - te).count();
            if (stats) {
                ctx->hstat.enqueue_s += d;
                if (d > ctx->hstat.enqueue_max_s) ctx->hstat.enqueue_max_s = d;
            }
        }
        if (rc == 0) rc = process(++*done);
    }
    if (rc != 0) {
        (void)hipStreamSynchronize(ctx->stream);
        return rc;
    }
    if (stats) host_stats_end(ctx);
    return 0;
}

struct ProxPlan {
    int M, N, batch;
    int tiles_i, tiles_j, nblk;
    int ftiles_i, ftiles_j, fnblk;
    int cj, nw, minw, rpl;
    ProxCtrl *ctrl;
    double *pbuf;
    int pairs;
    std::string tag;
    double *partials;
    size_t part_stride;
    unsigned *counters;
    const int *order;
    int esub_off;
};
int prox_plan(sbtv_ctx *ctx, int M, int N, int batch, ProxPlan *plan, const char *tag = "prox");
int prox_reset(sbtv_ctx *ctx, const ProxPlan &pl, const double *lambda_dev, double lambda_scale,
               int maxiter, double tol, double tau, bool keep_cur, const int *frozen);
int prox_zero_duals(sbtv_ctx *ctx, const ProxPlan &pl);
int prox_set_duals(sbtv_ctx *ctx, const ProxPlan &pl, const double *px, const double *py);
int prox_get_duals(sbtv_ctx *ctx, const ProxPlan &pl, double *px, double *py);
constexpr int FSMAX = 10;
constexpr double SPEC_TOL_GUARD = 1.0 + 1e-12;
constexpr double ESUB_MARGIN = 32.0;
constexpr int FSTRIDE = 32;
constexpr int SALSA_TAGS = 8 + FSTRIDE;
struct Collect {
    const double *acc;
    int nrb;
    const double *tvp;
    int ntv;
    const double *post;
    int npb;
    const double *ppart;
    int pnblk, psteps;
    unsigned long long psum_addr;
    const double *mse0;
};
struct SideJob {
    Collect c;
    unsigned long long out_addr, tags_addr;
    const int *frozen;
    double seq;
    int nblocks;
};
#ifdef __HIPCC__
#include "collect.inc"
#endif

int prox_iterate(sbtv_ctx *ctx, const ProxPlan &pl, const double *g, int maxiter, double *f_out = nullptr,
                 bool cold = false, int spec = 0, int spec_parity = 0, const SideJob *side = nullptr);
int prox_reserve_pairs(sbtv_ctx *ctx, ProxPlan *pl, int pairs);
int prox_launches(const ProxPlan &pl, int maxiter);
bool prox_spec_ok(const ProxPlan &pl, const double *g, const double *f_out, int maxiter);
constexpr double CHAMBOLLE_TOL = 1e-3, CHAMBOLLE_TAU = 0.249;

constexpr int SOLVE_RESTART_EXACT = 12345;
int spec_stop_rule(sbtv_ctx *ctx, ProxPlan &pp, const double *stepsums, int K, double tol, const int *frozen = nullptr);
template <class Body>
int solve_with_exact_repeat(sbtv_ctx *ctx, bool spec, Body &&body) {
    const long long calls0 = ctx->calls;
    const int rc = body(spec);
    if (rc != SOLVE_RESTART_EXACT) return rc;
    ctx->calls = calls0;
    ctx->solve_stats[0] += 1;
    return body(false);
}
int upload_frozen(sbtv_ctx *ctx, const int *frozen_h, int *frozen_d, int batch, ProxCtrl *park_ctrl);
int prox_finish(sbtv_ctx *ctx, const ProxPlan &pl, const double *g, double *f);
int tvnorm_dev(sbtv_ctx *ctx, const double *x, int M, int N, int batch, double *out_dev);
int tvnorm_partials(sbtv_ctx *ctx, const double *x, int M, int N, int batch, double **partials, int *nblk);

enum SpecOp {
    OP_NONE = 0,
    OP_MUL_H = 1,
    OP_MUL_HC = 2,
    OP_INVLS = 3,
    OP_SALSA = 4,
    OP_RESID = 5,
    OP_GRAD = 6,
    OP_ATA = 7,
    OP_GRADF = 8,
    OP_CSALSA = 9,
};
struct FftPlan {
    int M, N, batch;
    int n1;
    int wave;
    int u_tiled;
    size_t u_img;
    size_t s_img;
    int generic;
    const double2 *tw_n1;
    const double2 *tw_M;
    const double2 *tw_N;
};
int fft_plan(sbtv_ctx *ctx, int M, int N, int batch, FftPlan *plan);
int fft_cols_fwd(sbtv_ctx *ctx, const FftPlan &pl, const double *x, const double *add, double2 *S);
// ... 171 lines not shown
```

semi-blind-image-deblurring-problems-with-tv_amd/csrc/tv.hip:

```cpp
#include <mutex>

#include <algorithm>
#include "sbtv_internal.h"

#pragma clang fp contract(off)

namespace sbtv {

constexpr int TI = 128;
constexpr int TJ = 16;
constexpr int CJ = TJ / 4;
constexpr int ULD = TI + 2;
constexpr int TVB = 256;

__device__ __forceinline__ double wave_sum(double v) {
#pragma unroll
    for (int off = 32; off > 0; off >>= 1) v += __shfl_xor(v, off, 64);
    return v;
}

__device__ __forceinline__ double block_sum_256(double v, double *red ) {
    v = wave_sum(v);
    const int lane = threadIdx.x & 63, w = threadIdx.x >> 6;
    if (lane == 0) red[w] = v;
// ... 79 lines not shown
        if (c4 == 0 || c4 == CJ) {
            pym = (j > 0) ? ld2<VEC>(pyi, off - M, ok0, ok1) : make_double2(0.0, 0.0);
        }
        double pxm = __shfl_up(pxv.y, 1, 64);
        if (lane == 0) pxm = (i > 0 && ok0) ? pxi[off - 1] : 0.0;
        const double dx0 = div1(pxv.x, pxm, i, M);
        const double dx1 = div1(pxv.y, pxv.x, i + 1, M);
        const double dy0 = div1(pyv.x, pym.x, j, N);
        const double dy1 = div1(pyv.y, pym.y, j, N);
        double2 u;
        u.x = (dy0 + dx0) - gv.x / lambda;
        u.y = (dy1 + dx1) - gv.y / lambda;
        *reinterpret_cast<double2 *>(&u_lds[jl * ULD + il]) = u;
        if (c4 < CJ) {
            px[c4] = pxv;
            py[c4] = pyv;
        }
        pym = pyv;
    }
    if (w == 1 && lane < TJ) {
        const int ih = i0 + TI;
        const int j = j0 + lane;
        if (ih < M && j < N) {
            const size_t off = (size_t)j * M + ih;
            const double pxv = pxi[off], pxm = pxi[off - 1];
            const double pyv = pyi[off];
            const double pymv = (j > 0) ? pyi[off - M] : 0.0;
            const double dx = div1(pxv, pxm, ih, M);
            const double dy = div1(pyv, pymv, j, N);
            u_lds[lane * ULD + TI] = (dy + dx) - gg[off] / lambda;
        }
    }
    __syncthreads();

    double esum = 0.0;
#pragma unroll
    for (int c4 = 0; c4 < CJ; ++c4) {
        const int jl = w * CJ + c4;
        const int j = j0 + jl;
        if (j < N) {
            const double2 uc = *reinterpret_cast<const double2 *>(&u_lds[jl * ULD + il]);
            const double ud = u_lds[jl * ULD + il + 2];
            const double2 ur = *reinterpret_cast<const double2 *>(&u_lds[(jl + 1) * ULD + il]);
            const bool jin = (j < N - 1);
            const double upx0 = (i < M - 1) ? (uc.y - uc.x) : 0.0;
            const double upx1 = (i + 1 < M - 1) ? (ud - uc.y) : 0.0;
            const double upy0 = jin ? (ur.x - uc.x) : 0.0;
            const double upy1 = jin ? (ur.y - uc.y) : 0.0;
            const double t0 = sqrt(upx0 * upx0 + upy0 * upy0);
            const double t1 = sqrt(upx1 * upx1 + upy1 * upy1);
            if (ok0) {
                const double a = -upx0 + t0 * px[c4].x, bb = -upy0 + t0 * py[c4].x;
                esum += a * a + bb * bb;
            }
            if (ok1) {
                const double a = -upx1 + t1 * px[c4].y, bb = -upy1 + t1 * py[c4].y;
                esum += a * a + bb * bb;
            }
            double2 npx, npy;
            npx.x = (px[c4].x + tau * upx0) / (1.0 + tau * t0);
            npx.y = (px[c4].y + tau * upx1) / (1.0 + tau * t1);
            npy.x = (py[c4].x + tau * upy0) / (1.0 + tau * t0);
            npy.y = (py[c4].y + tau * upy1) / (1.0 + tau * t1);
            const size_t off = (size_t)j * M + i;
            st2<VEC>(pxo, off, npx, ok0, ok1);
            st2<VEC>(pyo, off, npy, ok0, ok1);
        }
    }
    const double bs = block_sum_256(esum, red);
    if (threadIdx.x == 0) partials[(size_t)b * (gridDim.x * gridDim.y) + (size_t)tj * tiles_i + ti] = bs;
}

constexpr int FH = 6;
constexpr int FHJ = 5;
constexpr int FHL = FHJ + 1;
constexpr int FRI = 128;
constexpr int FCI = FRI - 2 * FH;
constexpr int F1RI = 64;
constexpr int F1HT = FHJ + 1;
constexpr int F1HB = FHJ;
constexpr int F1CI = F1RI - F1HT - F1HB;
struct alignas(16) FusedStagger {
    int stagger;
};
static int fused_stagger(int nblk) {
    static const int v = [] {
        const char *e = getenv("SBTV_FUSED_STAGGER");
        return e ? atoi(e) : 6;
    }();
    return nblk >= 3 * 256 ? v : 0;
}
struct FusedVariant { int cj; int nw; int minw; int fast; int rpl; };
static FusedVariant g_fused = {4, 8, 4, 1, 2};
static bool g_fused_forced = false;

__device__ __forceinline__ double dpp_from_prev_lane(double v) {
    int lo = __double2loint(v), hi = __double2hiint(v);
    lo = __builtin_amdgcn_update_dpp(0, lo, 0x138, 0xf, 0xf, true);
    hi = __builtin_amdgcn_update_dpp(0, hi, 0x138, 0xf, 0xf, true);
    return __hiloint2double(hi, lo);
}
__device__ __forceinline__ double dpp_from_next_lane(double v) {
    int lo = __double2loint(v), hi = __double2hiint(v);
    lo = __builtin_amdgcn_update_dpp(0, lo, 0x130, 0xf, 0xf, true);
    hi = __builtin_amdgcn_update_dpp(0, hi, 0x130, 0xf, 0xf, true);
    return __hiloint2double(hi, lo);
}

__device__ __forceinline__ void fused_store_partial(double *p, double v) {
    __hip_atomic_store(p, v, __ATOMIC_RELAXED, __HIP_MEMORY_SCOPE_AGENT);
}

__device__ __forceinline__ void fused_reduce_steps(const double *__restrict__ partials_b, int nblk, int nsteps,
                                                   double *__restrict__ tots ) {
    const int nwaves = blockDim.x >> 6, lane = threadIdx.x & 63;
    for (int s = threadIdx.x >> 6; s < nsteps; s += nwaves) {
        const double *p = partials_b + (size_t)s * nblk;
        double acc = 0.0;
        for (int base = 0; base < nblk; base += 64 * 16) {
            double v[16];
#pragma unroll
            for (int r = 0; r < 16; ++r) {
                const int q = base + r * 64 + lane;
                v[r] = (q < nblk) ? __hip_atomic_load(p + q, __ATOMIC_RELAXED, __HIP_MEMORY_SCOPE_AGENT) : 0.0;
            }
#pragma unroll
            for (int r = 0; r < 16; ++r) acc += v[r];
        }
        acc = wave_sum(acc);
        if (lane == 0) tots[s] = acc;
    }
    __syncthreads();
}

__device__ __forceinline__ void fused_apply_stop_rule(ProxCtrl *c, const double *tots, int nsteps, int write_f) {
    for (int s = 0; s < nsteps; ++s) {
        const int k = c->k + s + 1;
        const double err = sqrt(tots[s]);
        const bool stop = !((k < c->maxiter) && (err > c->tol));
        if (stop) {
            c->done = 1;
            if (s == nsteps - 1) {
                c->k = k;
                c->err = err;
                c->cur ^= 1;
                if (write_f) c->f_valid = 1;
            } else {
                c->redo = s + 1;
            }
            return;
        }
    }
    c->k += nsteps;
    c->err = sqrt(tots[nsteps - 1]);
    c->cur ^= 1;
    if (write_f && c->k >= c->maxiter) c->f_valid = 1;
}

__device__ __forceinline__ void fused_inline_ctrl(ProxCtrl *__restrict__ c, const double *__restrict__ partials_b,
                                                  int nblk, int nsteps, int write_f,
                                                  unsigned *__restrict__ counter_b, int redo_mode) {
    __shared__ double ic_tots[FSMAX];
    __shared__ int ic_last;
    asm volatile("s_waitcnt vmcnt(0)" ::: "memory");
    __syncthreads();
    if (threadIdx.x == 0) {
        const unsigned t = __hip_atomic_fetch_add(counter_b, 1u, __ATOMIC_RELAXED, __HIP_MEMORY_SCOPE_AGENT);
        const int last = (t == gridDim.x - 1) ? 1 : 0;
        if (last) {
            __builtin_amdgcn_fence(__ATOMIC_ACQUIRE, "agent");
            asm volatile("s_waitcnt vmcnt(0)" ::: "memory");
        }
        ic_last = last;
// ... 280 lines not shown

__global__ __launch_bounds__(256) void reduce_jobs_kernel(RedJobs jb) {
    __shared__ double red[4];
    int v = blockIdx.x, q = 0;
    while (q < 3 && v >= jb.nvec[q]) v -= jb.nvec[q++];
    const int n = jb.n[q];
    const double *p = jb.src[q] + (size_t)v * n;
    double s = 0.0;
    for (int i = threadIdx.x; i < n; i += 256) s += p[i];
    const double tot = block_sum_256(s, red);
    if (threadIdx.x == 0) jb.dst[q][v] = tot;
}

__global__ void copy_duals_kernel(double *__restrict__ dst0, double *__restrict__ dst1,
                                  const double *__restrict__ pbuf, const ProxCtrl *__restrict__ ctrl, size_t P,
                                  int batch) {
    const int b = blockIdx.y;
    const ProxCtrl c = ctrl[b];
    const size_t plane = P * batch;
    const double *px = pbuf + (size_t)((c.cur & 1) * 2 + 0) * plane + (size_t)b * P;
    const double *py = pbuf + (size_t)((c.cur & 1) * 2 + 1) * plane + (size_t)b * P;
    for (size_t q = (size_t)blockIdx.x * blockDim.x + threadIdx.x; q < P; q += (size_t)gridDim.x * blockDim.x) {
        dst0[(size_t)b * P + q] = px[q];
        dst1[(size_t)b * P + q] = py[q];
    }
}


static inline bool vec_ok(const void *p, int M) { return (M % 2 == 0) && ((reinterpret_cast<uintptr_t>(p) & 15) == 0); }

int prox_plan(sbtv_ctx *ctx, int M, int N, int batch, ProxPlan *pl, const char *tag) {
    pl->M = M;
    pl->N = N;
    pl->batch = batch;
    pl->tiles_i = (M + TI - 1) / TI;
    pl->tiles_j = (N + TJ - 1) / TJ;
    pl->nblk = pl->tiles_i * pl->tiles_j;
    {
        static std::once_flag env_once;
        std::call_once(env_once, [] {
            if (const char *e = getenv("SBTV_FUSED_VARIANT")) {
                int cj = 0, nw = 0, mw = 0, rpl = 2;
                static const int known[][4] = {{4, 8, 4, 2}, {4, 8, 4, 1}};
                bool ok = false;
                if (sscanf(e, "%d,%d,%d,%d", &cj, &nw, &mw, &rpl) >= 3)
                    for (auto &k4 : known) ok = ok || (k4[0] == cj && k4[1] == nw && k4[2] == mw && k4[3] == rpl);
                if (ok) {
                    g_fused_forced = true;
                    g_fused.cj = cj;
                    g_fused.nw = nw;
                    g_fused.minw = mw;
                    g_fused.rpl = rpl;
                }
            }
            if (getenv("SBTV_EXACT") != nullptr) g_fused.fast = 0;
        });
    }
    auto geometry = [&](int cj, int nw, int rpl) {
        const int core_rows = (rpl == 1) ? F1CI : FCI, core_cols = cj * nw - FHL - FHJ;
        pl->ftiles_i = (M + core_rows - 1) / core_rows;
        pl->ftiles_j = (N + core_cols - 1) / core_cols;
        pl->fnblk = pl->ftiles_i * pl->ftiles_j;
        pl->cj = cj;
        pl->nw = nw;
        pl->rpl = rpl;
    };
    geometry(g_fused.cj, g_fused.nw, g_fused.rpl);
    pl->minw = g_fused.minw;
    if (!g_fused_forced && (size_t)pl->fnblk * batch < 256) {
        geometry(4, 8, 1);
        pl->minw = 4;
    }
    pl->esub_off = 0;
    const size_t P = (size_t)M * N;
    size_t npart = (size_t)batch * pl->nblk;
    if ((size_t)batch * FSTRIDE * pl->fnblk > npart) npart = (size_t)batch * FSTRIDE * pl->fnblk;
    const std::string t(tag ? tag : "prox");
    SBTV_TRY(ws_get_t(ctx, (t + ".ctrl").c_str(), (size_t)batch, &pl->ctrl));
    SBTV_TRY(ws_get_t(ctx, (t + ".pbuf").c_str(), 4 * P * batch, &pl->pbuf));
    pl->pairs = 2;
    pl->tag = t;
    SBTV_TRY(ws_get_t(ctx, (t + ".partials").c_str(), 2 * npart, &pl->partials));
    pl->part_stride = npart;
    pl->order = nullptr;
    {
        static const bool env_off = [] {
            const char *e = getenv("SBTV_TILE_ORDER");
            return e && e[0] == '0';
        }();
        const int nt = pl->fnblk;
        if (!env_off && pl->rpl == 2 && nt > 2 * 256) {
            int *od = nullptr;
            const std::string name = "prox.order." + std::to_string(M) + "x" + std::to_string(N) + "." + std::to_string(pl->cj) +
                                     "." + std::to_string(pl->nw);
            const bool built = ctx->ws.find(name) != ctx->ws.end();
            SBTV_TRY(ws_get_t(ctx, name.c_str(), (size_t)nt, &od));
            if (!built) {
                std::vector<int> h(nt);
                const int q8 = nt >> 3, r8 = nt & 7, ti_n = pl->ftiles_i, tj_n = pl->ftiles_j;
                for (int x = 0; x < 8; ++x) {
                    const int c0 = (x < r8 ? x * (q8 + 1) : r8 * (q8 + 1) + (x - r8) * q8);
                    const int len = q8 + (x < r8 ? 1 : 0);
                    int o = 0;
                    static const int env_mode = [] {
                        const char *e = getenv("SBTV_TILE_ORDER");
                        return e ? atoi(e) : 1;
                    }();
                    std::vector<int> chunk;
                    for (int t2 = c0; t2 < c0 + len; ++t2) chunk.push_back(t2);
                    if (env_mode >= 2)
                        std::stable_sort(chunk.begin(), chunk.end(), [&](int a, int b2) { return (a % ti_n) < (b2 % ti_n); });
                    for (int pass = 0; pass < 2; ++pass)
                        for (int t2 : chunk) {
                            const int ti = t2 % ti_n, tj = t2 / ti_n;
                            const bool border = (ti == 0 || ti == ti_n - 1 || tj == 0 || tj == tj_n - 1);
                            if (env_mode == 3 ? (pass == 0) : (border == (pass == 0))) h[(size_t)(o++) * 8 + x] = t2;
                        }
                }
                SBTV_HIP(ctx, hipStreamSynchronize(ctx->stream));
                SBTV_HIP(ctx, hipMemcpy(od, h.data(), sizeof(int) * nt, hipMemcpyHostToDevice));
            }
            pl->order = od;
        }
    }
    SBTV_TRY(ws_get_t(ctx, (t + ".counters").c_str(), (size_t)batch, &pl->counters));
    SBTV_HIP(ctx, hipMemsetAsync(pl->counters, 0, sizeof(unsigned) * batch, ctx->stream));
    return 0;
}

int prox_reserve_pairs(sbtv_ctx *ctx, ProxPlan *pl, int pairs) {
    if (pairs <= pl->pairs) return 0;
    if (pairs > 15) return fail(ctx, SBTV_ERR_BADARG, "prox_reserve_pairs: at most 15 dual buffers");
    const size_t P = (size_t)pl->M * pl->N;
    SBTV_TRY(ws_get_t(ctx, (pl->tag + ".pbuf").c_str(), (size_t)2 * pairs * P * pl->batch, &pl->pbuf));
    pl->pairs = pairs;
    return 0;
}

int prox_reset(sbtv_ctx *ctx, const ProxPlan &pl, const double *lambda_dev, double lambda_scale, int maxiter,
               double tol, double tau, bool keep_cur, const int *frozen) {
    const int thr = 64;
    hipLaunchKernelGGL(prox_reset_kernel, dim3((pl.batch + thr - 1) / thr), dim3(thr), 0, ctx->stream, pl.ctrl,
                       lambda_dev, lambda_scale, maxiter, tol, tau, keep_cur ? 1 : 0, pl.batch, frozen);
    SBTV_HIP(ctx, hipGetLastError());
    return 0;
}

int prox_zero_duals(sbtv_ctx *ctx, const ProxPlan &pl) {
    const size_t P = (size_t)pl.M * pl.N;
    SBTV_HIP(ctx, hipMemsetAsync(pl.pbuf, 0, 2 * P * pl.batch * sizeof(double), ctx->stream));
    return 0;
}

int prox_set_duals(sbtv_ctx *ctx, const ProxPlan &pl, const double *px, const double *py) {
    const size_t P = (size_t)pl.M * pl.N * pl.batch;
    SBTV_HIP(ctx, hipMemcpyAsync(pl.pbuf, px, P * sizeof(double), hipMemcpyDeviceToDevice, ctx->stream));
    SBTV_HIP(ctx, hipMemcpyAsync(pl.pbuf + P, py, P * sizeof(double), hipMemcpyDeviceToDevice, ctx->stream));
    return 0;
}

int prox_get_duals(sbtv_ctx *ctx, const ProxPlan &pl, double *px, double *py) {
    const size_t P = (size_t)pl.M * pl.N;
    hipLaunchKernelGGL(copy_duals_kernel, dim3(256, pl.batch), dim3(256), 0, ctx->stream, px, py, pl.pbuf, pl.ctrl,
                       P, pl.batch);
    SBTV_HIP(ctx, hipGetLastError());
    return 0;
}

int g_force_single_step = 0;

int prox_finish(sbtv_ctx *ctx, const ProxPlan &pl, const double *g, double *f);

bool prox_spec_ok(const ProxPlan &pl, const double *g, const double *f_out, int maxiter) {
    static const bool env_single = (getenv("SBTV_SINGLE_STEP") != nullptr);
    static const bool env_off = [] {
        const char *e = getenv("SBTV_PROX_SPEC");
        return e && e[0] == '0';
    }();
    return !env_off && !env_single && !g_force_single_step && maxiter <= FSTRIDE && vec_ok(g, pl.M) &&
           vec_ok(pl.pbuf, pl.M) && (!f_out || vec_ok(f_out, pl.M));
}

int prox_launches(const ProxPlan &pl, int maxiter) {
    return (maxiter + FHJ - 1) / FHJ;
}

int prox_iterate(sbtv_ctx *ctx, const ProxPlan &pl, const double *g, int maxiter, double *f_out, bool cold, int spec,
                 int spec_parity, const SideJob *side) {
    const bool spec_cur = spec != 0;
    const bool mb = spec >= 2;
    const bool mb_main = spec != 4, mb_ctrl = spec == 2, mb_redo = spec == 2 || spec == 4;
    if (mb && (!cold || !f_out || (size_t)pl.pairs < (size_t)prox_launches(pl, maxiter) + 2))
        return fail(ctx, SBTV_ERR_BADARG, "prox_iterate: the multi-buffer mode needs a cold prox with f output and prox_reserve_pairs()");
    const dim3 grid(pl.tiles_i, pl.tiles_j, pl.batch);
    const bool v = vec_ok(g, pl.M) && vec_ok(pl.pbuf, pl.M);
    static const bool env_single = (getenv("SBTV_SINGLE_STEP") != nullptr);
    if (spec_cur && !prox_spec_ok(pl, g, f_out, maxiter))
        return fail(ctx, SBTV_ERR_BADARG, "prox_iterate: optimistic mode is not available for this plan");
    if (v && !env_single && !g_force_single_step && (!f_out || vec_ok(f_out, pl.M))) {
        dim3 fgrid(pl.fnblk, 1, pl.batch);
        const SideJob no_side{};
        const int nl = prox_launches(pl, maxiter);
        const int base = maxiter / nl, extra = maxiter % nl;
        static const char *env_inl = getenv("SBTV_INLINE_CTRL");
        const bool env_inline = env_inl ? (env_inl[0] != '0') : ((size_t)pl.fnblk * pl.batch <= 512);
        int spec_off = 0, spec_l = 0;
        auto launch_fused = [&](int steps, int redo, int write_f) -> int {
            bool launched = false;
            const SideJob &sj = (spec_cur && side && spec_l == 0) ? *side : no_side;
            fgrid.x = pl.fnblk + sj.nblocks;
            const int inl = (!redo && env_inline && !spec_cur) ? 1 : 0;
            int kflags = inl | (cold ? 2 : 0);
            if (spec_cur) {
                if (mb && redo) {
                    kflags = 4 | 8 | 2 | ((nl + 1) << 24);
                } else if (mb) {
                    kflags = 4 | 8 | 2 | (spec_off << 12) | (spec_l << 20) | ((spec_l + 1) << 24);
                } else {
                    kflags = 4 | (cold ? 2 : 0) | ((spec_l & 1) << 8) | ((spec_parity & 1) << 9) | (spec_off << 12);
                }
                if (!redo) {
                    ++spec_l;
                    spec_off += steps;
                }
            }
#define SBTV_FUSED_CASE(CJ_, NW_, MW_)                                                                               \
    if (pl.rpl == 2 && pl.cj == CJ_ && pl.nw == NW_ && pl.minw == MW_) {                         \
        launched = true;                                                                                             \
        if (g_fused.fast)                                                                                            \
            hipLaunchKernelGGL((chambolle_fused_kernel<CJ_, NW_, MW_, true>), fgrid, dim3(64 * NW_), 0, ctx->stream, \
                               g, pl.pbuf, pl.ctrl, pl.partials, pl.M, pl.N, pl.batch, pl.ftiles_i, pl.fnblk, steps, \
                               redo, f_out, write_f, pl.counters, kflags, sj, pl.order, FusedStagger{fused_stagger(pl.fnblk)});  \
        else                                                                                                         \
            hipLaunchKernelGGL((chambolle_fused_kernel<CJ_, NW_, MW_, false>), fgrid, dim3(64 * NW_), 0,             \
                               ctx->stream, g, pl.pbuf, pl.ctrl, pl.partials, pl.M, pl.N, pl.batch, pl.ftiles_i,     \
                               pl.fnblk, steps, redo, f_out, write_f, pl.counters, kflags, sj, pl.order, FusedStagger{fused_stagger(pl.fnblk)}); \
    }
            static const bool esub_wanted = [] {
                const char *e = getenv("SBTV_ERR_SUBSET");
                return !(e && e[0] == '0');
            }();
            if (esub_wanted && !pl.esub_off && spec == 1 && !redo && pl.rpl == 2 && pl.cj == 4 && pl.nw == 8 && pl.minw == 4 &&
                g_fused.fast) {
                launched = true;
                hipLaunchKernelGGL((chambolle_fused_kernel<4, 8, 4, true, true>), fgrid, dim3(64 * 8), 0, ctx->stream, g, pl.pbuf,
                                   pl.ctrl, pl.partials, pl.M, pl.N, pl.batch, pl.ftiles_i, pl.fnblk, steps, redo, f_out, write_f,
                                   pl.counters, kflags, sj, pl.order, FusedStagger{fused_stagger(pl.fnblk)});
            } else
            SBTV_FUSED_CASE(4, 8, 4)
#undef SBTV_FUSED_CASE
#define SBTV_FUSED1_CASE(CJ_, NW_, MW_)                                                                              \
    if (pl.rpl == 1 && pl.cj == CJ_ && pl.nw == NW_ && pl.minw == MW_) {                         \
        launched = true;                                                                                             \
        if (g_fused.fast)                                                                                            \
            hipLaunchKernelGGL((chambolle_fused1_kernel<CJ_, NW_, MW_, true>), fgrid, dim3(64 * NW_), 0,             \
                               ctx->stream, g, pl.pbuf, pl.ctrl, pl.partials, pl.M, pl.N, pl.batch, pl.ftiles_i,     \
                               pl.fnblk, steps, redo, f_out, write_f, pl.counters, kflags, sj);                         \
        else                                                                                                         \
            hipLaunchKernelGGL((chambolle_fused1_kernel<CJ_, NW_, MW_, false>), fgrid, dim3(64 * NW_), 0,            \
                               ctx->stream, g, pl.pbuf, pl.ctrl, pl.partials, pl.M, pl.N, pl.batch, pl.ftiles_i,     \
                               pl.fnblk, steps, redo, f_out, write_f, pl.counters, kflags, sj);                         \
    }
            if (esub_wanted && !pl.esub_off && spec == 1 && !redo && pl.rpl == 1 && pl.cj == 4 && pl.nw == 8 && pl.minw == 4 && g_fused.fast) {
                launched = true;
                hipLaunchKernelGGL((chambolle_fused1_kernel<4, 8, 4, true, true>), fgrid, dim3(64 * 8), 0, ctx->stream, g, pl.pbuf,
                                   pl.ctrl, pl.partials, pl.M, pl.N, pl.batch, pl.ftiles_i, pl.fnblk, steps, redo, f_out, write_f,
                                   pl.counters, kflags, sj);
            } else
            SBTV_FUSED1_CASE(4, 8, 4)
#undef SBTV_FUSED1_CASE
            if (!launched)
                return fail(ctx, SBTV_ERR_BADARG, "prox_iterate: no fused Chambolle kernel is compiled for this tile geometry");
            if (!inl && !redo && !spec_cur)
                hipLaunchKernelGGL(chambolle_fused_ctrl_kernel, dim3(pl.batch), dim3(64 * FSMAX), 0, ctx->stream,
                                   pl.ctrl, pl.partials, pl.fnblk, steps, redo, write_f);
            return 0;
        };
        const int wf = f_out ? 1 : 0;
        if (mb_main)
            for (int l = 0; l < nl; ++l) SBTV_TRY(launch_fused(base + (l < extra ? 1 : 0), 0, (l == nl - 1) ? wf : 0));
        if (mb && mb_ctrl)
            hipLaunchKernelGGL(chambolle_mb_ctrl_kernel, dim3(pl.batch), dim3(64 * FSMAX), 0, ctx->stream, pl.ctrl, pl.partials,
                               pl.fnblk, maxiter, base, extra);
        if (mb && mb_redo) SBTV_TRY(launch_fused(0, 1, wf));
        if (!spec_cur) SBTV_TRY(launch_fused(0, 1, wf));
        SBTV_HIP(ctx, hipGetLastError());
        return 0;
    }
    if (cold) SBTV_TRY(prox_zero_duals(ctx, pl));
    for (int it = 0; it < maxiter; ++it) {
        if (v)
            hipLaunchKernelGGL(chambolle_iter_kernel<true>, grid, dim3(TVB), 0, ctx->stream, g, pl.pbuf, pl.ctrl,
                               pl.partials, pl.M, pl.N, pl.batch, pl.tiles_i);
        else
            hipLaunchKernelGGL(chambolle_iter_kernel<false>, grid, dim3(TVB), 0, ctx->stream, g, pl.pbuf, pl.ctrl,
                               pl.partials, pl.M, pl.N, pl.batch, pl.tiles_i);
        hipLaunchKernelGGL(chambolle_ctrl_kernel, dim3(pl.batch), dim3(256), 0, ctx->stream, pl.ctrl, pl.partials,
                           pl.nblk);
    }
    SBTV_HIP(ctx, hipGetLastError());
    if (f_out) return prox_finish(ctx, pl, g, f_out);
    return 0;
}

int prox_finish(sbtv_ctx *ctx, const ProxPlan &pl, const double *g, double *f) {
    const dim3 grid(pl.tiles_i, pl.tiles_j, pl.batch);
    const bool v = vec_ok(g, pl.M) && vec_ok(pl.pbuf, pl.M) && vec_ok(f, pl.M);
    if (v)
        hipLaunchKernelGGL(chambolle_finish_kernel<true>, grid, dim3(TVB), 0, ctx->stream, g, pl.pbuf, pl.ctrl, f,
                           pl.M, pl.N, pl.batch);
    else
        hipLaunchKernelGGL(chambolle_finish_kernel<false>, grid, dim3(TVB), 0, ctx->stream, g, pl.pbuf, pl.ctrl, f,
                           pl.M, pl.N, pl.batch);
    SBTV_HIP(ctx, hipGetLastError());
    return 0;
}

int reduce_jobs(sbtv_ctx *ctx, const RedJobs &jb) {
    if (jb.dropped) return fail(ctx, SBTV_ERR_BADARG, "reduce_jobs: more than four jobs in one launch (a reduction would be skipped)");
    int tot = 0;
    for (int q = 0; q < 4; ++q) tot += jb.nvec[q];
    if (tot <= 0) return 0;
    hipLaunchKernelGGL(reduce_jobs_kernel, dim3(tot), dim3(256), 0, ctx->stream, jb);
    SBTV_HIP(ctx, hipGetLastError());
    return 0;
}

int reduce_partials(sbtv_ctx *ctx, const double *partials, int nvec, int n, double *out) {
    hipLaunchKernelGGL(reduce_partials_kernel, dim3(nvec), dim3(256), 0, ctx->stream, partials, n, out);
    SBTV_HIP(ctx, hipGetLastError());
// ... 32 lines not shown
int sbtv_chambolle_prox_TV_stop(sbtv_ctx *ctx, const double *g, int M, int N, int batch, const double *lambda,
                                int maxiter, double tol, double tau, int warm_start, double *px, double *py,
                                double *f, int *k_out, double *err_out, int flags) {
    if (!ctx) return SBTV_ERR_BADARG;
    if (!g || !lambda || M < 2 || N < 2 || batch < 1)
        return fail(ctx, SBTV_ERR_BADARG, "chambolle_prox_TV_stop: Wrong number of required parameters");
    if (maxiter <= 0)
        return fail(ctx, SBTV_ERR_MAXITER,
                    "chambolle_prox_TV_stop: 'maxiter' is required (MaxIter undefined, chambolle_prox_TV_stop.m:131)");
    if (warm_start && (!px || !py))
        return fail(ctx, SBTV_ERR_DUALVARS, "chambolle_prox_TV_stop: Wrong size of the dual variables");
    SBTV_HIP(ctx, hipSetDevice(ctx->device));
    const size_t cnt = (size_t)M * N * batch;
    ProxPlan pl;
    SBTV_TRY(prox_plan(ctx, M, N, batch, &pl));
    const double *gd = nullptr;
    SBTV_TRY(stage_in(ctx, "prox.in.g", g, cnt, flags, &gd));
    double *lam_d = nullptr;
    SBTV_TRY(ws_get_t(ctx, "prox.lambda", (size_t)batch, &lam_d));
    SBTV_HIP(ctx, hipMemcpyAsync(lam_d, lambda, sizeof(double) * batch, hipMemcpyHostToDevice, ctx->stream));
    SBTV_TRY(prox_reset(ctx, pl, lam_d, 1.0, maxiter, tol, tau, false, nullptr));
    if (warm_start) {
        const double *pxd = nullptr, *pyd = nullptr;
        SBTV_TRY(stage_in(ctx, "prox.in.px", px, cnt, flags, &pxd));
        SBTV_TRY(stage_in(ctx, "prox.in.py", py, cnt, flags, &pyd));
        SBTV_TRY(prox_set_duals(ctx, pl, pxd, pyd));
    }
    double *fd = nullptr, *pxo = nullptr, *pyo = nullptr;
    if (f) SBTV_TRY(stage_out_buf(ctx, "prox.out.f", f, cnt, flags, &fd));
    SBTV_TRY(prox_iterate(ctx, pl, gd, maxiter, fd, !warm_start));
    if (f) SBTV_TRY(stage_out_copy(ctx, f, fd, cnt, flags));
    if (px && py) {
        SBTV_TRY(stage_out_buf(ctx, "prox.out.px", px, cnt, flags, &pxo));
        SBTV_TRY(stage_out_buf(ctx, "prox.out.py", py, cnt, flags, &pyo));
        SBTV_TRY(prox_get_duals(ctx, pl, pxo, pyo));
        SBTV_TRY(stage_out_copy(ctx, px, pxo, cnt, flags));
        SBTV_TRY(stage_out_copy(ctx, py, pyo, cnt, flags));
    }
    if (k_out || err_out || !(flags & SBTV_DEVICE_PTRS)) {
        std::vector<ProxCtrl> hc(batch);
        SBTV_HIP(ctx, hipMemcpyAsync(hc.data(), pl.ctrl, sizeof(ProxCtrl) * batch, hipMemcpyDeviceToHost, ctx->stream));
        SBTV_HIP(ctx, hipStreamSynchronize(ctx->stream));
        for (int b = 0; b < batch; ++b) {
            if (k_out) k_out[b] = hc[b].k;
            if (err_out) err_out[b] = hc[b].err;
        }
    }
    return canary_epilogue(ctx, 0);
}

int sbtv_diag_prox_variant(sbtv_ctx *ctx, int M, int N, int batch, int out[6]) {
    if (!ctx || !out || M < 2 || N < 2 || batch < 1) return SBTV_ERR_BADARG;
    SBTV_HIP(ctx, hipSetDevice(ctx->device));
    ProxPlan pl;
    SBTV_TRY(prox_plan(ctx, M, N, batch, &pl));
    static const bool env_single = (getenv("SBTV_SINGLE_STEP") != nullptr);
    out[0] = pl.cj;
    out[1] = pl.nw;
    out[2] = pl.minw;
    out[3] = pl.rpl;
    out[4] = pl.fnblk;
    out[5] = (M % 2 == 0 && !env_single && !g_force_single_step) ? 1 : 0;
    return 0;
}

int sbtv_diag_prox_geometry(sbtv_ctx *ctx, int M, int N, int batch, int out[16]) {
    if (!ctx || !out || M < 2 || N < 2 || batch < 1) return SBTV_ERR_BADARG;
    SBTV_HIP(ctx, hipSetDevice(ctx->device));
    ProxPlan pl;
    SBTV_TRY(prox_plan(ctx, M, N, batch, &pl));
    const bool two = (pl.rpl == 2);
    out[0] = two ? FRI : F1RI;
    out[1] = two ? FCI : F1CI;
    out[2] = two ? FH : F1HT;
    out[3] = two ? FH : F1HB;
    out[4] = pl.rpl;
    out[5] = pl.cj * pl.nw;
    out[6] = pl.cj * pl.nw - FHL - FHJ;
    out[7] = FHL;
    out[8] = FHJ;
    out[9] = pl.ftiles_i;
    out[10] = pl.ftiles_j;
    out[11] = pl.order != nullptr ? 1 : 0;
    out[12] = two ? fused_stagger(pl.fnblk) : 0;
    out[13] = TI;
    out[14] = TJ;
    out[15] = FHJ;
    return 0;
}

int sbtv_TVnorm(sbtv_ctx *ctx, const double *x, int M, int N, int batch, double *out, int flags) {
    if (!ctx) return SBTV_ERR_BADARG;
    if (!x || !out || M < 2 || N < 2 || batch < 1) return fail(ctx, SBTV_ERR_BADARG, "TVnorm: bad arguments");
    SBTV_HIP(ctx, hipSetDevice(ctx->device));
    const double *xd = nullptr;
    SBTV_TRY(stage_in(ctx, "tv.in.x", x, (size_t)M * N * batch, flags, &xd));
    double *od = nullptr;
    SBTV_TRY(ws_get_t(ctx, "tv.out", (size_t)batch, &od));
    SBTV_TRY(tvnorm_dev(ctx, xd, M, N, batch, od));
    SBTV_HIP(ctx, hipMemcpyAsync(out, od, sizeof(double) * batch, hipMemcpyDeviceToHost, ctx->stream));
    SBTV_HIP(ctx, hipStreamSynchronize(ctx->stream));
    return canary_epilogue(ctx, 0);
}

}

#ifdef SBTV_FUSED_TIMELINE
extern "C" int sbtv_debug_timeline(sbtv_ctx *ctx, unsigned long long *out, int nrec) {
    if (!ctx || !out || nrec < 1 || nrec > 8192) return SBTV_ERR_BADARG;
    SBTV_HIP(ctx, hipStreamSynchronize(ctx->stream));
    SBTV_HIP(ctx, hipMemcpyFromSymbol(out, HIP_SYMBOL(sbtv::g_fused_tl), sizeof(unsigned long long) * 8 * (size_t)nrec));
    return 0;
}
extern "C" int sbtv_debug_timeline_waves(sbtv_ctx *ctx, unsigned long long *out, int *samples, int *every, int *slots) {
    if (!ctx || !out) return SBTV_ERR_BADARG;
    SBTV_HIP(ctx, hipStreamSynchronize(ctx->stream));
    SBTV_HIP(ctx, hipMemcpyFromSymbol(out, HIP_SYMBOL(sbtv::g_fused_tlw), sizeof(sbtv::g_fused_tlw)));
    if (samples) *samples = sbtv::TLW_SAMPLES;
    if (every) *every = sbtv::TLW_EVERY;
    if (slots) *slots = sbtv::TLW_SLOTS;
    return 0;
}
#endif
```

semi-blind-image-deblurring-problems-with-tv_amd/csrc/tv_fused.inc:

```

#ifndef SBTV_FUSED_SCHED_FREE_MAX_CJ
#define SBTV_FUSED_SCHED_FREE_MAX_CJ 0
#endif

#ifndef SBTV_DIET
#define SBTV_DIET 3
#endif
__device__ __forceinline__ double fused_rcp(double d) {
    double r = __builtin_amdgcn_rcp(d);
    double e = __builtin_fma(-d, r, 1.0);
#if SBTV_DIET & 1
    return __builtin_fma(r, __builtin_fma(e, e, e), r);
#else
    r = __builtin_fma(r, e, r);
    e = __builtin_fma(-d, r, 1.0);
    r = __builtin_fma(r, e, r);
    return r;
#endif
}

constexpr double FUSED_TINY = 1e-300;
__device__ __forceinline__ double fused_sqrt(double s) {
    const double y = __builtin_amdgcn_rsq(s);
#if SBTV_DIET & 2
// ... 284 lines not shown
        double2 gvv[FCJ];
#pragma unroll
        for (int q = 0; q < FCJ; ++q)
            gvv[q] = *reinterpret_cast<const double2 *>(gg + (size_t)min(max(jw + q, 0), N - 1) * M + min(max(gi, 0), M - 2));
#pragma unroll
        for (int q = 0; q < FCJ; ++q) {
            const int cl = w * FCJ + q;
            const int gj = jw + q;
            const double pxm = dpp_from_prev_lane(px[q].y);
            const double2 pyl = (q > 0) ? py[q > 0 ? q - 1 : 0] : pyl0;
            if (rcore && rin && cl >= FHL && cl < FRJ - FHJ && (INTERIOR || (gj >= 0 && gj < N))) {
                double dx0, dx1, dy0, dy1;
                if (INTERIOR) {
                    dx0 = px[q].x - pxm;
                    dx1 = px[q].y - px[q].x;
                    dy0 = py[q].x - pyl.x;
                    dy1 = py[q].y - pyl.y;
                } else {
                    dx0 = div1(px[q].x, pxm, gi, M);
                    dx1 = div1(px[q].y, px[q].x, gi + 1, M);
                    dy0 = div1(py[q].x, pyl.x, gj, N);
                    dy1 = div1(py[q].y, pyl.y, gj, N);
                }
                const size_t off = (size_t)gj * M + gi;
                const double2 gv = gvv[q];
                *reinterpret_cast<double2 *>(f_out + off) =
                    make_double2(gv.x - lambda * (dy0 + dx0), gv.y - lambda * (dy1 + dx1));
            }
        }
    }
    for (int s = w; s < nsteps; s += FNW) {
        double acc = 0.0;
#pragma unroll
        for (int ww = 0; ww < FNW; ++ww) acc += esl[s][ww * 64 + lane];
        const double tot = wave_sum(acc);
        if (lane == 0) fused_store_partial(&partial_out[(size_t)s * nblk], tot);
    }
    SBTV_TL(3);
}

template <int FCJ, int FNW, int MINW, bool FAST, bool ESUB = false>
__global__ __launch_bounds__(64 * FNW, MINW) void chambolle_fused_kernel(const double *__restrict__ g,
                                                                          double *__restrict__ pbuf,
                                                                          ProxCtrl *__restrict__ ctrl,
                                                                          double *__restrict__ partials, int M, int N,
                                                                          int batch, int tiles_i, int nblk,
                                                                          int steps_arg, int redo_mode,
                                                                          double *__restrict__ f_all, int write_f,
                                                                          unsigned *__restrict__ counters,
                                                                          int inline_ctrl, SideJob side,
                                                                          const int *__restrict__ order, FusedStagger stg) {
    constexpr int FRJ = FCJ * FNW;
    const int b = blockIdx.z;
    const int nside = side.nblocks;
    if ((int)blockIdx.x < nside) {
        __shared__ double sred[4];
        salsa_collect_block(side.c, nullptr, side.out_addr, side.frozen, 0, side.tags_addr, side.seq, blockIdx.x, b, sred);
        return;
    }
    const ProxCtrl c = ctrl[b];
    const bool spec = (inline_ctrl & 4) != 0, mb = (inline_ctrl & 8) != 0;
    int nsteps;
    if (spec && !redo_mode) {
        if (c.done) return;
        nsteps = steps_arg;
    } else if (redo_mode) {
        if (c.redo <= 0 && (c.f_valid || !f_all)) return;
        nsteps = c.redo > 0 ? c.redo : 0;
    } else {
        if (c.done) return;
        nsteps = min(steps_arg, c.maxiter - c.k);
        if (nsteps <= 0) return;
    }
    const size_t P = (size_t)M * N;
    const size_t plane = P * batch;
    const bool cold = (inline_ctrl & 2) && (mb && redo_mode ? (c.cur == 0) : spec ? (((inline_ctrl >> 12) & 31) == 0) : (c.k == 0));
    const int src = mb ? (redo_mode ? c.cur : ((inline_ctrl >> 20) & 15)) : ((c.cur ^ (spec ? ((inline_ctrl >> 8) ^ (inline_ctrl >> 9)) : 0)) & 1);
    const int dst = mb ? ((inline_ctrl >> 24) & 15) : (src ^ 1);
    const double *pxi = cold ? nullptr : pbuf + (size_t)(src * 2 + 0) * plane + (size_t)b * P;
    const double *pyi = cold ? nullptr : pbuf + (size_t)(src * 2 + 1) * plane + (size_t)b * P;
    double *pxo = pbuf + (size_t)(dst * 2 + 0) * plane + (size_t)b * P;
    double *pyo = pbuf + (size_t)(dst * 2 + 1) * plane + (size_t)b * P;
    const double *gg = g + (size_t)b * P;
    __shared__ __attribute__((aligned(16))) double lds[(FRJ + 2 * FNW) * FRI + FH * 64 * FNW];
    int tile;
    {
        const int nt = gridDim.x - nside, bid = blockIdx.x - nside;
        const int q8 = nt >> 3, r8 = nt & 7, x = bid & 7, o = bid >> 3;
        tile = (x < r8 ? x * (q8 + 1) : r8 * (q8 + 1) + (x - r8) * q8) + o;
        if (order) tile = order[bid];
    }
    double *fo = (write_f && f_all) ? f_all + (size_t)b * P : nullptr;
    const int stagger = stg.stagger;
    if (stagger > 0) {
        const int bid = blockIdx.x - nside;
        if (bid >= 256 && bid < 512 && b == 0)
            for (int q = 0; q < stagger; ++q) __builtin_amdgcn_s_sleep(18);
    }
    const int ti = tile % tiles_i, tj = tile / tiles_i;
    double *pout = partials + ((size_t)b * FSTRIDE + (spec ? ((inline_ctrl >> 12) & 31) : 0)) * nblk + (size_t)tj * tiles_i + ti;
    const int i0 = ti * FCI - FH, j0 = tj * (FRJ - FHL - FHJ) - FHL;
    const bool interior = (i0 >= 1) && (i0 + FRI <= M - 1) && (j0 >= 1) && (j0 + FRJ <= N - 1);
    if (interior)
        fused_body<FCJ, FNW, FAST, true, ESUB>(gg, pxi, pyi, pxo, pyo, pout, nblk, M, N, ti, tj, nsteps, c.lambda, c.tau, lds,
                                               fo);
    else
        fused_body<FCJ, FNW, FAST, false, ESUB>(gg, pxi, pyi, pxo, pyo, pout, nblk, M, N, ti, tj, nsteps, c.lambda, c.tau,
                                                lds, fo);
    if (!spec && ((inline_ctrl & 1) || redo_mode))
        fused_inline_ctrl(&ctrl[b], partials + (size_t)b * FSTRIDE * nblk, nblk, nsteps, write_f, counters + b, redo_mode);
}
```

semi-blind-image-deblurring-problems-with-tv_amd/sbtv/_lib.py:

```python
from __future__ import annotations

import ctypes as C
import os
import threading

import numpy as np

_HERE = os.path.dirname(os.path.abspath(__file__))
LIB_PATH = os.environ.get("SBTV_LIBRARY") or os.path.join(os.path.dirname(_HERE), "lib", "libsbtv.so")

SBTV_HOST_PTRS = 0
SBTV_DEVICE_PTRS = 1

ERRORS = {
    -1: "SBTV_ERR_BADARG", -2: "SBTV_ERR_SIZE", -3: "SBTV_ERR_MAXITER", -4: "SBTV_ERR_DUALVARS",
    -5: "SBTV_ERR_MODE", -6: "SBTV_ERR_STOPCRITERION", -7: "SBTV_ERR_INIT", -8: "SBTV_ERR_MISSING_AT",
    -9: "SBTV_ERR_MISSING_LS", -10: "SBTV_ERR_PSF", -11: "SBTV_ERR_NOMEM", -12: "SBTV_ERR_NODEVICE",
    -13: "SBTV_ERR_CANARY", -14: "SBTV_ERR_PEER",
}


class SbtvError(RuntimeError):
    def __init__(self, code, msg):
        super().__init__(f"[{ERRORS.get(code, code)}] {msg}")
# ... 72 lines not shown
FISTA_EXACT_PROX = 2

_P = C.c_void_p
_D = C.c_double
_I = C.c_int

SIGNATURES = {
    "sbtv_version": (_I, []),
    "sbtv_ctx_create": (_I, [_I, C.POINTER(_P)]),
    "sbtv_ctx_destroy": (_I, [_P]),
    "sbtv_last_error": (C.c_char_p, [_P]),
    "sbtv_ctx_set_stream": (_I, [_P, _P]),
    "sbtv_ctx_sync": (_I, [_P]),
    "sbtv_ctx_set_lanes": (_I, [_P, _I]),
    "sbtv_callcounter_get": (_I, [_P, C.POINTER(C.c_longlong)]),
    "sbtv_callcounter_reset": (_I, [_P]),
    "sbtv_last_timing": (_I, [_P, C.POINTER(_D)]),
    "sbtv_malloc": (_I, [_P, C.c_size_t, C.POINTER(_P)]),
    "sbtv_free": (_I, [_P, _P]),
    "sbtv_memcpy_h2d": (_I, [_P, _P, _P, C.c_size_t]),
    "sbtv_memcpy_d2h": (_I, [_P, _P, _P, C.c_size_t]),
    "sbtv_chambolle_prox_TV_stop": (_I, [_P, _P, _I, _I, _I, _P, _I, _D, _D, _I, _P, _P, _P, _P, _P, _I]),
    "sbtv_TVnorm": (_I, [_P, _P, _I, _I, _I, _P, _I]),
    "sbtv_A_wrapper": (_I, [_P, _P, _I, _P, _P, _P, _I, _I, _I, _I, _I]),
    "sbtv_psf_taps": (_I, [_I, _I, _P, _P, _P, _P]),
    "sbtv_err_psf": (_I, [_I, _I, _P, _I, _P, _D, _P]),
    "sbtv_rfft2_packed": (_I, [_P, _P, _P, _I, _I, _I, _I, _I]),
    "sbtv_salsa_opts_default": (None, [C.POINTER(sbtv_salsa_opts)]),
    "sbtv_SALSA_v2": (_I, [_P, _P, _I, _I, _I, _P, _I, _P, _P, C.POINTER(sbtv_salsa_opts), _P, _P, _P, _P, _P, _P,
                           _P, _P, _P, _P, _I]),
    "sbtv_CSALSA_v2": (_I, [_P, _P, _I, _I, _I, _P, _I, _P, _P, _P, _P, _D, C.POINTER(sbtv_salsa_opts), _P, _P, _P,
                            _P, _P, _P, _P, _P, _P, _P, _P, _P, _I]),
    "sbtv_CoRAL_v2": (_I, [_P, _P, _I, _I, _I, _P, _I, _P, _P, _P, _P, _P, _I, C.POINTER(sbtv_salsa_opts), _P, _P, _P,
                           _P, _P, _P, _P, _P, _P, _P, _I]),
    "sbtv_SALSA_masked": (_I, [_P, _P, _P, _I, _I, _I, _P, _I, _P, _P, _P, C.POINTER(sbtv_salsa_opts), _P, _P, _P, _P, _P,
                               _P, _P, _P, _P, _P, _I]),
    "sbtv_mrdwt_TI2D": (_I, [_P, _P, _I, _I, _I, _P, _I, _I, _P, _I]),
    "sbtv_mirdwt_TI2D": (_I, [_P, _P, _I, _I, _I, _P, _I, _I, _P, _I]),
    "sbtv_soft": (_I, [_P, _P, _I, _I, _I, _P, _P, _I]),
    "sbtv_SALSA_wavelet": (_I, [_P, _P, _I, _I, _I, _P, _I, _P, _I, _I, _P, _P, C.POINTER(sbtv_salsa_opts), _P, _P, _P, _P,
                                _P, _P, _P, _P, _P, _P, _P, _I]),
    "sbtv_SAPG_wavelet": (_I, [_P, _P, _I, _I, _I, _P, _I, _P, _I, _I, C.POINTER(sbtv_sapg_wavelet_opts), _P, _P, _P, _P, _P,
                               _P, _P, _P, _P, _P, _I]),
    "sbtv_SAPG_wavelet_semiblind": (_I, [_P, _P, _I, _I, _I, _P, _I, _I, C.POINTER(sbtv_sapg_wavelet_sb_opts), _P, _P, _P, _P,
                                         _P, _P, _P, _P, _P, _P, _P, _P, _P, _P, _P, _P, _I]),
    "sbtv_fista_tv": (_I, [_P, _P, _I, _I, _I, _P, _I, _P, _D, _I, _I, _D, _I, _I, _P, _P, _P, _P, _P, _I]),
    "sbtv_SAPG_algorithm": (_I, [_P, _P, _I, _I, _I, C.POINTER(sbtv_sapg_opts), _P, _P, _P, _P, _P, _P, _P, _P, _P,
                                 _P, _P, ALLREDUCE_FN, _P, _I]),
    "sbtv_SAPG_algorithm_moments": (_I, [_P, _P, _I, _I, _I, C.POINTER(sbtv_sapg_opts), _P, _P, _P, _P, _P, _P, _P, _P,
                                         _P, _P, _P, ALLREDUCE_FN, _P, C.POINTER(sbtv_moments_opts), _P, _P, _P, _I]),
    "sbtv_myula": (_I, [_P, _P, _I, _I, _I, _P, _I, _D, _D, _P, _P, _I, _I, C.c_ulonglong, _I, _P, _P, _I]),
    "sbtv_myula_moments": (_I, [_P, _P, _I, _I, _I, _P, _I, _D, _D, _P, _P, _I, _I, C.c_ulonglong, _I, _P, _P,
                                C.POINTER(sbtv_moments_opts), _P, _P, _P, _I]),
    "sbtv_myula_wavelet": (_I, [_P, _P, _I, _I, _I, _P, _I, _P, _I, _I, C.POINTER(sbtv_myula_wavelet_opts), _P, _P, _P, _P, _P,
                                _P, _P, C.POINTER(sbtv_moments_opts), _P, _P, _P, _P, _P, _I]),
    "sbtv_max_eigenval": (_I, [_P, _P, _I, _P, _I, _I, _D, _I, _P, _P, _I]),
    "sbtv_PSNR": (_I, [_P, _P, _P, _I, _I, _I, _P, _I]),
    "sbtv_MSE": (_I, [_P, _P, _P, _I, _I, _I, _P, _I]),
    "sbtv_group_create": (_I, [C.POINTER(_I), _I, C.POINTER(_P)]),
    "sbtv_group_destroy": (_I, [_P]),
    "sbtv_group_size": (_I, [_P]),
    "sbtv_group_ctx": (_P, [_P, _I]),
    "sbtv_group_last_error": (C.c_char_p, [_P]),
    "sbtv_group_shard_of": (_I, [_P, _I, _I, C.POINTER(_I), C.POINTER(_I), C.POINTER(_I)]),
    "sbtv_SALSA_v2_sharded": (_I, [_P, _P, _I, _I, _I, _P, _I, _P, _P, C.POINTER(sbtv_salsa_opts), _P, _P, _P, _P, _P,
                                   _P, _P, _P, _P, _P]),
    "sbtv_SALSA_v2_sharded_dev": (_I, [_P, _P, _I, _I, _I, _P, _I, _P, _P, C.POINTER(sbtv_salsa_opts), _P, _P, _P, _P, _P,
                                       _P, _P, _P, _P, _P]),
    "sbtv_SAPG_algorithm_sharded": (_I, [_P, _P, _I, _I, _I, C.POINTER(sbtv_sapg_opts), _P, _P, _P, _P, _P, _P, _P, _P,
                                         _P, _P, _P]),
    "sbtv_fista_tv_sharded": (_I, [_P, _P, _I, _I, _I, _P, _I, _P, _D, _I, _I, _D, _I, _I, _P, _P, _P, _P, _P]),
    "sbtv_CSALSA_v2_sharded": (_I, [_P, _P, _I, _I, _I, _P, _I, _P, _P, _P, _P, _D, C.POINTER(sbtv_salsa_opts), _P, _P,
                                    _P, _P, _P, _P, _P, _P, _P, _P, _P, _P]),
    "sbtv_CoRAL_v2_sharded": (_I, [_P, _P, _I, _I, _I, _P, _I, _P, _P, _P, _P, _P, _I, C.POINTER(sbtv_salsa_opts), _P,
                                   _P, _P, _P, _P, _P, _P, _P, _P, _P]),
    "sbtv_SALSA_masked_sharded": (_I, [_P, _P, _P, _I, _I, _I, _P, _I, _P, _P, _P, C.POINTER(sbtv_salsa_opts), _P, _P, _P,
                                       _P, _P, _P, _P, _P, _P, _P]),
    "sbtv_diag_stage_stats": (_I, [_P, C.POINTER(_D)]),
    "sbtv_host_transpose": (_I, [_P, _P, _I, _I, _I]),
    "sbtv_diag_solve_stats": (_I, [_P, C.POINTER(_D)]),
    "sbtv_diag_canary": (_I, [_P, _I, C.POINTER(_I), C.POINTER(_I), C.POINTER(_I)]),
    "sbtv_diag_prox_variant": (_I, [_P, _I, _I, _I, C.POINTER(_I)]),
    "sbtv_diag_prox_geometry": (_I, [_P, _I, _I, _I, C.POINTER(_I)]),
    "sbtv_diag_fft_plan": (_I, [_P, _I, _I, _I, C.POINTER(_I)]),
    "sbtv_diag_spectral_pass": (_I, [_P, C.POINTER(sbtv_diag_pass)]),
    "sbtv_last_host_stats": (_I, [_P, C.POINTER(_D)]),
    "sbtv_diag_workspace": (_I, [_P, C.c_char_p, C.POINTER(_P), C.POINTER(C.c_size_t)]),
    "sbtv_diag_switches": (_I, [C.c_char_p, C.c_size_t]),
    "sbtv_diag_time_pass": (_I, [_P, _I, _I, _I, _I, _I, C.POINTER(_D), C.POINTER(_D)]),
}

_lib = None
_lib_lock = threading.Lock()


def load_library():
    global _lib
    with _lib_lock:
        if _lib is not None:
            return _lib
        try:
            import torch
        except ImportError:
            pass
        if not os.path.exists(LIB_PATH):
            raise ImportError(
                f"{LIB_PATH} not found: build it with __graft_entry__.build() (hipcc --offload-arch=gfx950). "
                "sbtv has no CPU fallback.")
        lib = C.CDLL(LIB_PATH)
        for name, (res, args) in SIGNATURES.items():
            fn = getattr(lib, name)
            fn.restype = res
            fn.argtypes = args
        _lib = lib
        return lib


class Context:

    def __init__(self, device: int = 0):
        self.lib = load_library()
        h = _P()
        rc = self.lib.sbtv_ctx_create(int(device), C.byref(h))
        if rc != 0:
            raise SbtvError(rc, self.lib.sbtv_last_error(None).decode())
        self.h = h
        self.device = int(device)

    def close(self):
        if getattr(self, "h", None):
            self.lib.sbtv_ctx_destroy(self.h)
            self.h = None

    def __del__(self):
        try:
            self.close()
        except Exception:
            pass

    def check(self, rc, flags=0):
        if rc != 0:
            raise SbtvError(rc, self.lib.sbtv_last_error(self.h).decode())
        if flags & SBTV_DEVICE_PTRS:
            self.sync()

    def sync(self):
        self.check(self.lib.sbtv_ctx_sync(self.h))

    def set_lanes(self, mode):
        self.check(self.lib.sbtv_ctx_set_lanes(self.h, int(mode)))

    def solve_stats(self):
        out = (C.c_double * 4)()
        self.check(self.lib.sbtv_diag_solve_stats(self.h, out))
        return dict(exact_restarts=int(out[0]), esub_off=int(out[1]))

    def stage_stats(self):
        out = (C.c_double * 4)()
        self.check(self.lib.sbtv_diag_stage_stats(self.h, out))
        return dict(bytes_in=out[0], s_in=out[1], bytes_out=out[2], s_out=out[3])

    def set_stream(self, stream_ptr):
        self.check(self.lib.sbtv_ctx_set_stream(self.h, _P(stream_ptr)))

    @property
    def calls(self):
        v = C.c_longlong(0)
        self.check(self.lib.sbtv_callcounter_get(self.h, C.byref(v)))
        return v.value

    def reset_calls(self):
        self.check(self.lib.sbtv_callcounter_reset(self.h))

    def canary(self, poke=False):
        en, nb, bad = _I(0), _I(0), _I(0)
        self.check(self.lib.sbtv_diag_canary(self.h, int(bool(poke)), C.byref(en), C.byref(nb), C.byref(bad)))
        return dict(enabled=bool(en.value), buffers=nb.value, bad_bytes=bad.value)

    PASSES = {"cols_fwd": 0, "rows_salsa": 1, "cols_inv_post": 2, "cols_inv": 3, "rows_fwd": 4, "rows_grad": 5,
              "rows_gradf": 6, "prox10_warm": 7, "prox25_cold": 8,
              "fused_steps1": 11, "fused_steps2": 12, "fused_steps3": 13, "fused_steps4": 14, "fused_steps5": 15}

    def time_pass(self, name, M, N, batch=1, reps=20):
        ms, by = _D(0.0), _D(0.0)
        self.check(self.lib.sbtv_diag_time_pass(self.h, self.PASSES[name], int(M), int(N), int(batch), int(reps),
                                                C.byref(ms), C.byref(by)))
        return dict(ms=ms.value, bytes=by.value, gbs=by.value / (ms.value * 1e-3) / 1e9 if ms.value > 0 else 0.0)

    def prox_variant(self, M, N, batch=1):
        out = (_I * 6)()
        self.check(self.lib.sbtv_diag_prox_variant(self.h, int(M), int(N), int(batch), out))
        return dict(cols_per_wave=out[0], waves=out[1], waves_per_simd=out[2], rows_per_lane=out[3], tiles=out[4],
                    fused=bool(out[5]), kind={0: "single-step", 1: "tile", 2: "pipeline"}[out[5]])

    GEOMETRY = ("region_rows", "core_rows", "halo_top", "halo_bottom", "rows_per_lane", "region_cols", "core_cols",
                "halo_left", "halo_right", "tiles_i", "tiles_j", "order", "stagger", "single_ti", "single_tj", "max_steps")

    def prox_geometry(self, M, N, batch=1):
        out = (_I * 16)()
        self.check(self.lib.sbtv_diag_prox_geometry(self.h, int(M), int(N), int(batch), out))
        g = dict(zip(self.GEOMETRY, out))
        g["order"] = bool(g["order"])
        return g

    FFT_PLAN = ("generic", "wave", "n1", "cols_per_wg", "cols_threads", "cols_wgs", "rows_per_wg", "rows_threads",
                "rows_wgs", "rows_kind", "u_tiled", "L_M", "L_N", "lch", "fold", "caps")

    def fft_plan(self, M, N, batch=1):
        out = (_I * 16)()
        self.check(self.lib.sbtv_diag_fft_plan(self.h, int(M), int(N), int(batch), out))
        p = dict(zip(self.FFT_PLAN, out))
        caps = p.pop("caps")
        for k in ("generic", "wave", "u_tiled", "fold"):
            p[k] = bool(p[k])
        p["rows_kind"] = {0: "workgroup", 1: "pipelined", 2: "pointwise"}[p["rows_kind"]]
        p.update(tv_ok=bool(caps & 1), step_ok=bool(caps & 2), csalsa_ok=bool(caps & 4))
        return p

    SPEC_OPS = {"none": 0, "mul_h": 1, "mul_hc": 2, "invls": 3, "salsa": 4, "resid": 5, "grad": 6, "ata": 7, "gradf": 8,
                "csalsa": 9}
    EPILOGUES = {"plain": 0, "post": 1, "step": 2, "sub": 3, "post_skip_x": 4}

    def spectral_pass(self, x, op="none", epilogue="plain", taps=None, d1taps=None, d2taps=None, y=None, mu=None,
                      cs=None, e0=None, add=None, shared_spec=False, repeats=1, frozen=None, u=None, bu=None, bu_in=None,
                      tru=None, xprev=None, ystep=None, alpha=0.0, sub_b=None, tv=False, sentinel=0.0):
        def cm(a, lead=None):
            if a is None:
                return None
            a = np.asarray(a, dtype=np.float64)
            if a.ndim == 2:
                a = a[None]
            if lead is not None and a.shape[0] != lead:
                raise ValueError("leading dimension %d, expected %d" % (a.shape[0], lead))
            return np.ascontiguousarray(np.transpose(a, (0, 2, 1)))
        xc = cm(x)
        B, N, M = xc.shape
        ns = 1 if shared_spec else B
        keep = [xc]
        a = sbtv_diag_pass()
        a.M, a.N, a.batch = M, N, B
        a.op = self.SPEC_OPS[op] if isinstance(op, str) else int(op)
        a.epilogue = self.EPILOGUES[epilogue] if isinstance(epilogue, str) else int(epilogue)
        a.shared_spec, a.repeats, a.alpha = int(bool(shared_spec)), int(repeats), float(alpha)
        a.x = vptr(xc)
        tc = cm(taps, ns)
        a.taille = tc.shape[1] if tc is not None else 0
        for name, arr in (("add", cm(add, B)), ("taps", tc), ("d1taps", cm(d1taps, ns)), ("d2taps", cm(d2taps, ns)),
                          ("y", cm(y, ns)), ("e0", cm(e0, ns)), ("u", cm(u, B)), ("bu_in", cm(bu_in, B)),
                          ("tru", cm(tru, B)), ("xprev", cm(xprev, B)), ("sub_b", cm(sub_b, B))):
            if arr is not None:
                keep.append(arr)
                setattr(a, name, vptr(arr))
        for name, arr, n in (("mu", mu, B), ("cs", cs, 3)):
            if arr is not None:
                v = np.ascontiguousarray(np.broadcast_to(np.asarray(arr, dtype=np.float64), (n,)))
                keep.append(v)
                setattr(a, name, vptr(v))
        if frozen is not None:
            fz = np.ascontiguousarray(np.asarray(frozen, dtype=np.int32).reshape(B))
            keep.append(fz)
            a.frozen = vptr(fz)
        out = {}
        ep = a.epilogue
        if ep in (0, 1, 3):
            out["x"] = np.full((B, N, M), float(sentinel))
            a.x_out = vptr(out["x"])
        if ep in (1, 3, 4):
            out["g"] = np.full((B, N, M), float(sentinel))
            a.g_out = vptr(out["g"])
        if ep in (1, 4):
            out["sums"] = np.zeros((B, 6))
            a.sums = vptr(out["sums"])
            if bu is not None:
                out["bu"] = cm(bu, B)
                a.bu = vptr(out["bu"])
        if ep == 2 and ystep is not None:
            out["ystep"] = cm(ystep, B)
            a.ystep = vptr(out["ystep"])
        out["acc"] = np.zeros((B, 3))
        a.acc = vptr(out["acc"])
        if tv:
            out["tv"] = np.zeros(B)
            a.tv = vptr(out["tv"])
        self.check(self.lib.sbtv_diag_spectral_pass(self.h, C.byref(a)))
# ... 216 lines not shown
```

semi-blind-image-deblurring-problems-with-tv_amd/sbtv/salsa.py:

```python
from __future__ import annotations

import ctypes as C
import sys

import numpy as np

from . import _lib as L
from .operators import BlurOperator, _Adjoint, _InvLS
from .tv import _parse_varargin

_OPTIONS = {"P", "PT", "PSI", "PHI", "TVINITIALIZATION", "TVITERS", "MU", "STOPCRITERION", "TOLERANCEA",
            "MAXITERA", "INITIALIZATION", "TRUE_X", "AT", "VERBOSE", "LS", "SEED", "SPECULATE"}


def SALSA_v2(y, A, tau, *varargin, ctx=None, **kw):
    opts = _parse_varargin(varargin, _OPTIONS)
    for k, v in kw.items():
        opts[k.upper()] = v
    ctx = ctx or L.default_context()
    AT = opts.get("AT", 0)
    LS = opts.get("LS", None)
    mu = opts.get("MU", 1e-3)
    if not isinstance(A, BlurOperator):
        if not callable(A):
            raise TypeError("A must be a sbtv.BlurOperator or a function handle (a matrix A is not supported)")
        if not callable(AT):
            raise L.SbtvError(-8, "The function handle for transpose of A is missing")
        if not callable(LS):
            raise L.SbtvError(-9, "(A^T A + \\mu I)^(-1) must be specified as a function handle.")
        shape = tuple(y.shape[-2:])
        like = y if L._is_torch(y) else None
        A = BlurOperator.from_handle(A, shape, like=like, ctx=ctx)
        A.check_adjoint_handle(AT, shape, like=like)
        AT, LS = A.T, A.LS(A.mu_of_handle(LS, shape, like=like))
    if not isinstance(AT, _Adjoint) or AT.op is not A:
        raise L.SbtvError(-8, "The function handle for transpose of A is missing")
    if not isinstance(LS, _InvLS) or LS.op is not A:
        raise L.SbtvError(-9, "(A^T A + \\mu I)^(-1) must be specified as a function handle.")
    if "MU" not in opts:
        mu = LS.mu
    elif (abs(mu - LS.mu) > 1e-6 * abs(LS.mu)) if (isinstance(mu, float) and isinstance(LS.mu, float)) else \
            not np.allclose(np.asarray(mu, dtype=np.float64), np.asarray(LS.mu, dtype=np.float64), rtol=1e-6, atol=0.0):
        raise L.SbtvError(-9, "'MU' differs from the mu the 'LS' filter was built with: the GPU path has one mu "
                              "(run_Gaussian_demo.m:219-225 passes the same value to both)")
    if ("P" in opts) != ("PT" in opts):
        raise ValueError("If you give P you must also give PT, and vice versa.")
    if "P" in opts:
        raise NotImplementedError("'P'/'PT' other than the identity are not supported")
    if not opts.get("TVINITIALIZATION", 0):
        raise NotImplementedError("only the TV path ('TVINITIALIZATION', 1) runs on the GPU")
    if "PSI" in opts:
        print("Warning: user specified Phi and Psi will not be used as TV with initialization flag has been set to 1.",
              file=sys.stdout)
    so = L.sbtv_salsa_opts()
    ctx.lib.sbtv_salsa_opts_default(C.byref(so))
    so.stopcriterion = int(opts.get("STOPCRITERION", 1))
    if so.stopcriterion not in (1, 2, 3):
        raise L.SbtvError(-6, "Unknown stopping criterion")
    so.maxiter = int(opts.get("MAXITERA", 10000))
    so.TViters = int(opts.get("TVITERS", 5))
    so.tolA = float(opts.get("TOLERANCEA", 0.001))
    so.speculate = int(opts.get("SPECULATE", so.speculate))
    yi = L.Images(y)
    B, M, N = yi.B, yi.M, yi.N
    init = opts.get("INITIALIZATION", 0)
    xinit = None
    if np.ndim(init) > 0 or L._is_torch(init):
        xinit = L.Images(init)
        so.initialization = 33333
    else:
        so.initialization = int(init)
        if so.initialization == 1:
            rng = np.random.default_rng(int(opts.get("SEED", 0)))
            x0 = rng.standard_normal((yi.B, yi.M, yi.N))
            xinit = L.Images(L.to_device(x0, yi.t.device) if yi.torch else x0)
            so.initialization = 33333
        elif so.initialization not in (0, 2):
            raise L.SbtvError(-7, "Unknown 'Initialization' option")
    true = opts.get("TRUE_X", None)
    ti = L.Images(true) if true is not None else None
    if ti is not None and (ti.M, ti.N) != (M, N):
        raise ValueError("Initial x has incompatible size")
    so.compute_mse = 1 if ti is not None else 0
    for other in (xinit, ti):
        if other is not None and other.flags != yi.flags:
            raise ValueError("all image arguments must live in the same memory space")
    xo = L.empty_like_images(yi)
    K = so.maxiter
    objective = np.zeros((B, K + 1))
    distance = np.zeros((B, K))
    times = np.zeros((B, K + 1))
    mses = np.zeros((B, K + 1))
    numA = (C.c_int * B)()
    numAt = (C.c_int * B)()
    nout = (C.c_int * B)()
    taps = A._cm(B)
    tau_a, tau_p = L.dvec(tau, B)
    mu_a, mu_p = L.dvec(mu, B)
    vp = L.vptr
    if getattr(ctx, "is_group", False):
        if yi.flags != L.SBTV_HOST_PTRS:
            raise ValueError("a sbtv.Group takes host (NumPy) images")
        ctx.check(ctx.lib.sbtv_SALSA_v2_sharded(ctx.h, yi.ptr, M, N, B, vp(taps), A.taille, tau_p, mu_p, C.byref(so),
                                                ti.ptr if ti else None, xinit.ptr if xinit else None, xo.ptr,
                                                vp(objective), vp(distance), vp(times), vp(mses) if ti else None,
                                                numA, numAt, nout))
    else:
        ctx.check(ctx.lib.sbtv_SALSA_v2(ctx.h, yi.ptr, M, N, B, vp(taps), A.taille, tau_p, mu_p, C.byref(so),
                                        ti.ptr if ti else None, xinit.ptr if xinit else None, xo.ptr,
                                        vp(objective), vp(distance), vp(times), vp(mses) if ti else None,
                                        numA, numAt, nout, yi.flags), yi.flags)
    sq = (y.dim() == 2) if yi.torch else yi.squeeze
    x = L.images_result(xo, sq)
    n = np.array(nout[:])
    if sq or B == 1:
        k = int(n[0])
        return (x, int(numA[0]), int(numAt[0]), objective[0, :k + 1].copy(), distance[0, :k].copy(),
                times[0, :k + 1].copy(), mses[0, :k + 1].copy() if ti else np.array([]))
    return (x, np.array(numA[:]), np.array(numAt[:]), [objective[b, :n[b] + 1].copy() for b in range(B)],
            [distance[b, :n[b]].copy() for b in range(B)], [times[b, :n[b] + 1].copy() for b in range(B)],
            [mses[b, :n[b] + 1].copy() for b in range(B)] if ti else [])
```

Before: 4741 SALSA outer-iterations/s.

## Use wider 5-column tiles for speculative fused Chambolle prox

Adds a second tile geometry for the speculative fused Chambolle prox kernel that gives each wave 5 columns instead of 4. This yields fewer, wider tiles and less halo overhead per useful column, and a matching order table is built for it. Every consumer of the prox partial sums (SALSA, C-SALSA, ADMM, FISTA collect) now reads the tile count from the active geometry, and the stagger window is generalized to use the device CU count. The LDS array is resized by the column halo, and the wider tile raises per-block register and LDS pressure, which could lower occupancy.

Result: no change. 4762 SALSA outer-iterations/s, median of 4 (+0.4%).

```diff
diff --git a/include/sbtv.h b/include/sbtv.h
--- a/include/sbtv.h
+++ b/include/sbtv.h
@@ -306,6 +306,7 @@
 int sbtv_diag_time_pass(sbtv_ctx *ctx, int pass, int M, int N, int batch, int reps, double *ms_avg, double *alg_bytes);
 int sbtv_diag_prox_variant(sbtv_ctx *ctx, int M, int N, int batch, int out[6]);
 int sbtv_diag_prox_geometry(sbtv_ctx *ctx, int M, int N, int batch, int out[16]);
+int sbtv_diag_prox_spec_geometry(sbtv_ctx *ctx, int M, int N, int batch, int out[8]);
 int sbtv_diag_fft_plan(sbtv_ctx *ctx, int M, int N, int batch, int out[16]);
 typedef struct sbtv_diag_pass {
     int M, N, batch, op, epilogue, taille, shared_spec, repeats;
diff --git a/semi-blind-image-deblurring-problems-with-tv_amd/csrc/admm.hip b/semi-blind-image-deblurring-problems-with-tv_amd/csrc/admm.hip
--- a/semi-blind-image-deblurring-problems-with-tv_amd/csrc/admm.hip
+++ b/semi-blind-image-deblurring-problems-with-tv_amd/csrc/admm.hip
@@ -456,7 +456,7 @@
     }
     SBTV_TRY(prox_iterate(ctx, pp, g, K, f, false, 1, (int)(*nlaunch & 1), nullptr));
     *nlaunch += prox_launches(pp, K);
-    return reduce_partials(ctx, pp.partials, K, pp.fnblk, stepsums);
+    return reduce_partials(ctx, pp.partials, K, prox_spec_tiles(pp), stepsums);
 }
 
 struct AdmmSlots {
@@ -607,7 +607,7 @@
         } else {
             SBTV_TRY(prox_iterate(ctx, pp, g, K, u, false, 1, (int)(nlaunch & 1), nullptr));
             nlaunch += prox_launches(pp, K);
-            jb.add(pp.partials, K, pp.fnblk, sums + 16);
+            jb.add(pp.partials, K, prox_spec_tiles(pp), sums + 16);
         }
         hipLaunchKernelGGL(csalsa_post_kernel, dim3(nb), dim3(AB), 0, ctx->stream, xn, u, bu, td,
                            (opts->stopcriterion == 2) ? xprev : (const double *)nullptr, partials, (unsigned)M, (unsigned)N, P);
@@ -836,7 +836,7 @@
             } else {
                 SBTV_TRY(prox_iterate(ctx, pu, g1, K1, u, false, 1, (int)(nl_u & 1), nullptr));
                 nl_u += prox_launches(pu, K1);
-                jb.add(pu.partials, FSTRIDE + K1, pu.fnblk, sums + 16);
+                jb.add(pu.partials, FSTRIDE + K1, prox_spec_tiles(pu), sums + 16);
             }
         } else {
             SBTV_TRY(admm_prox(ctx, pu, g1, K1, u, sp, &nl_u, sums + 16, par + 1, opts->chambolle_tol, opts->chambolle_tau));
@@ -1033,7 +1033,7 @@
         } else {
             SBTV_TRY(prox_iterate(ctx, pp, g, K, u, false, 1, (int)(nlaunch & 1), nullptr));
             nlaunch += prox_launches(pp, K);
-            jb.add(pp.partials, K, pp.fnblk, sums + 16);
+            jb.add(pp.partials, K, prox_spec_tiles(pp), sums + 16);
         }
         {
             RowsArgs a{};
diff --git a/semi-blind-image-deblurring-problems-with-tv_amd/csrc/ctx.hip b/semi-blind-image-deblurring-problems-with-tv_amd/csrc/ctx.hip
--- a/semi-blind-image-deblurring-problems-with-tv_amd/csrc/ctx.hip
+++ b/semi-blind-image-deblurring-problems-with-tv_amd/csrc/ctx.hip
@@ -524,7 +524,7 @@
         "SBTV_CANARY", "SBTV_COLLECT_RIDE", "SBTV_EXACT", "SBTV_FFT_WAVE", "SBTV_FISTA_FUSED_STEP", "SBTV_FISTA_LAG",
         "SBTV_FUSED_VARIANT", "SBTV_GRAPH", "SBTV_INLINE_CTRL", "SBTV_PROX_SPEC", "SBTV_SAPG_DEFER",
         "SBTV_SAPG_FUSED_MYULA", "SBTV_SAPG_HOST", "SBTV_SINGLE_STEP", "SBTV_SPIN", "SBTV_TAG_SPIN_US", "SBTV_TILE_ORDER", "SBTV_SALSA_NOX", "SBTV_CSALSA_SPECTRAL",
-        "SBTV_CORAL_BATCH", "SBTV_ROWS_FOLD", "SBTV_ERR_SUBSET", "SBTV_LANES", "SBTV_LANE_COUNT", "SBTV_STAGE_THREADS", "SBTV_TEST_FAIL_SAPG", "SBTV_FUSED_STAGGER"};
+        "SBTV_CORAL_BATCH", "SBTV_ROWS_FOLD", "SBTV_ERR_SUBSET", "SBTV_LANES", "SBTV_LANE_COUNT", "SBTV_STAGE_THREADS", "SBTV_TEST_FAIL_SAPG", "SBTV_FUSED_STAGGER", "SBTV_FUSED_SPEC_COLS"};
     if (!buf || cap == 0) return SBTV_ERR_BADARG;
     std::string s;
     int nset = 0;
diff --git a/semi-blind-image-deblurring-problems-with-tv_amd/csrc/fista.hip b/semi-blind-image-deblurring-problems-with-tv_amd/csrc/fista.hip
--- a/semi-blind-image-deblurring-problems-with-tv_amd/csrc/fista.hip
+++ b/semi-blind-image-deblurring-problems-with-tv_amd/csrc/fista.hip
@@ -203,6 +203,7 @@
     const bool out_aliases_input = (flags & SBTV_DEVICE_PTRS) && (overlaps(bd, x_out, cnt) || overlaps(td, x_out, cnt));
     const bool prox_spec = spec_wanted && !out_aliases_input && prox_spec_ok(pp, y, x, prox_iters);
     bool prox_was_spec = false;
+    int prox_tiles = pp.fnblk;
     auto objective_of_x = [&](const double *xk, int k, const int *frozen, const double *mom_partials) -> int {
         RowsArgs a{};
         a.dir_fwd = 1;
@@ -223,7 +224,7 @@
         const int slot = k & 1;
         hipLaunchKernelGGL(fista_collect_kernel, dim3(prox_was_spec ? 7 + prox_iters : 7, batch), dim3(256), 0, ctx->stream,
                            (const double *)acc, nrb, mom_partials, npb, (const double *)tvp, ntv, scal_base_hd + slot * slot_n,
-                           batch, (const double *)pp.partials, pp.fnblk,
+                           batch, (const double *)pp.partials, prox_tiles,
                            (unsigned long long)(uintptr_t)(tags_base_hd + slot * slot_n), (double)k);
         SBTV_HIP(ctx, hipGetLastError());
         return 0;
@@ -285,6 +286,7 @@
             }
         }
         prox_was_spec = prox_spec;
+        prox_tiles = prox_spec ? prox_spec_tiles(pp) : pp.fnblk;
         slot_spec[k & 1] = prox_spec;
         SBTV_TRY(prox_iterate(ctx, pp, y, prox_iters, xk, true, prox_spec));
         t_enq = 0.5 * (1 + sqrt(1 + 4 * t_old * t_old));
diff --git a/semi-blind-image-deblurring-problems-with-tv_amd/csrc/salsa.hip b/semi-blind-image-deblurring-problems-with-tv_amd/csrc/salsa.hip
--- a/semi-blind-image-deblurring-problems-with-tv_amd/csrc/salsa.hip
+++ b/semi-blind-image-deblurring-problems-with-tv_amd/csrc/salsa.hip
@@ -256,6 +256,7 @@
         return !(e && e[0] == '0');
     }();
     bool slot_tagged[2] = {false, false}, slot_spec[2] = {false, false};
+    int slot_pnblk[2] = {pp.fnblk, pp.fnblk};
     long long prox_iters_timed = 0;
     struct PendingCollect {
         bool valid = false;
@@ -266,7 +267,8 @@
     const bool zero_start = (opts->initialization == 0);
     auto make_collect = [&](int outer, bool spec) -> Collect {
         const int slot = outer & 1;
-        return Collect{acc, nrb, nullptr, 0, postp, npb, spec ? pp.partials + (size_t)slot * pp.part_stride : nullptr, pp.fnblk,
+        return Collect{acc, nrb, nullptr, 0, postp, npb, spec ? pp.partials + (size_t)slot * pp.part_stride : nullptr,
+                       slot_pnblk[slot],
                        opts->TViters, (unsigned long long)(uintptr_t)(psum_hd + (size_t)slot * batch * FSTRIDE), nullptr};
     };
     auto launch_collect = [&](int outer, bool spec, bool tagged) -> int {
@@ -308,6 +310,7 @@
         if (timed) SBTV_HIP(ctx, hipEventRecord(ev_p0[slot], ctx->stream));
         ProxPlan pps = pp;
         pps.partials = pp.partials + (size_t)slot * pp.part_stride;
+        slot_pnblk[slot] = spec ? prox_spec_tiles(pps) : pp.fnblk;
         if (!(zero_start && outer == 1))
             SBTV_TRY(prox_iterate(ctx, pps, gb[(outer - 1) & 1], opts->TViters, u, outer == (zero_start ? 2 : 1), spec,
                                   spec ? ((outer - 2) * nl_prox) & 1 : 0, side.nblocks ? &side : nullptr));
diff --git a/semi-blind-image-deblurring-problems-with-tv_amd/csrc/sbtv_internal.h b/semi-blind-image-deblurring-problems-with-tv_amd/csrc/sbtv_internal.h
--- a/semi-blind-image-deblurring-problems-with-tv_amd/csrc/sbtv_internal.h
+++ b/semi-blind-image-deblurring-problems-with-tv_amd/csrc/sbtv_internal.h
@@ -384,7 +384,10 @@
     unsigned *counters;
     const int *order;
     int esub_off;
-};
+    int s_cj, s_tiles_i, s_tiles_j, s_nblk;
+    const int *s_order;
+};
+inline int prox_spec_tiles(const ProxPlan &pl) { return (pl.s_cj != pl.cj && !pl.esub_off) ? pl.s_nblk : pl.fnblk; }
 int prox_plan(sbtv_ctx *ctx, int M, int N, int batch, ProxPlan *plan, const char *tag = "prox");
 int prox_reset(sbtv_ctx *ctx, const ProxPlan &pl, const double *lambda_dev, double lambda_scale,
                int maxiter, double tol, double tau, bool keep_cur, const int *frozen);
diff --git a/semi-blind-image-deblurring-problems-with-tv_amd/csrc/tv.hip b/semi-blind-image-deblurring-problems-with-tv_amd/csrc/tv.hip
--- a/semi-blind-image-deblurring-problems-with-tv_amd/csrc/tv.hip
+++ b/semi-blind-image-deblurring-problems-with-tv_amd/csrc/tv.hip
@@ -185,13 +185,31 @@
 constexpr int F1CI = F1RI - F1HT - F1HB;
 struct alignas(16) FusedStagger {
     int stagger;
+    int lo, hi;
 };
-static int fused_stagger(int nblk) {
+constexpr int FUSED_STAGGER_CUS = 256;
+static FusedStagger fused_stagger(const sbtv_ctx *ctx, int nblk) {
     static const int v = [] {
         const char *e = getenv("SBTV_FUSED_STAGGER");
         return e ? atoi(e) : 6;
     }();
-    return nblk >= 3 * 256 ? v : 0;
+    const int cu = ctx->cu_count;
+    return FusedStagger{(cu == FUSED_STAGGER_CUS && nblk >= 3 * cu) ? v : 0, cu, 2 * cu};
+}
+constexpr int FUSED_SPEC_COLS_DEFAULT = 5;
+static int fused_spec_cols() {
+    static const int v = [] {
+        const char *e = getenv("SBTV_FUSED_SPEC_COLS");
+        return e ? atoi(e) : FUSED_SPEC_COLS_DEFAULT;
+    }();
+    return v;
+}
+static bool fused_esub_wanted() {
+    static const bool v = [] {
+        const char *e = getenv("SBTV_ERR_SUBSET");
+        return !(e && e[0] == '0');
+    }();
+    return v;
 }
 struct FusedVariant { int cj; int nw; int minw; int fast; int rpl; };
 static FusedVariant g_fused = {4, 8, 4, 1, 2};
@@ -638,46 +656,60 @@
     pl->tag = t;
     SBTV_TRY(ws_get_t(ctx, (t + ".partials").c_str(), 2 * npart, &pl->partials));
     pl->part_stride = npart;
-    pl->order = nullptr;
-    {
-        static const bool env_off = [] {
-            const char *e = getenv("SBTV_TILE_ORDER");
-            return e && e[0] == '0';
-        }();
-        const int nt = pl->fnblk;
-        if (!env_off && pl->rpl == 2 && nt > 2 * 256) {
-            int *od = nullptr;
-            const std::string name = "prox.order." + std::to_string(M) + "x" + std::to_string(N) + "." + std::to_string(pl->cj) +
-                                     "." + std::to_string(pl->nw);
-            const bool built = ctx->ws.find(name) != ctx->ws.end();
-            SBTV_TRY(ws_get_t(ctx, name.c_str(), (size_t)nt, &od));
-            if (!built) {
-                std::vector<int> h(nt);
-                const int q8 = nt >> 3, r8 = nt & 7, ti_n = pl->ftiles_i, tj_n = pl->ftiles_j;
-                for (int x = 0; x < 8; ++x) {
-                    const int c0 = (x < r8 ? x * (q8 + 1) : r8 * (q8 + 1) + (x - r8) * q8);
-                    const int len = q8 + (x < r8 ? 1 : 0);
-                    int o = 0;
-                    static const int env_mode = [] {
-                        const char *e = getenv("SBTV_TILE_ORDER");
-                        return e ? atoi(e) : 1;
-                    }();
-                    std::vector<int> chunk;
-                    for (int t2 = c0; t2 < c0 + len; ++t2) chunk.push_back(t2);
-                    if (env_mode >= 2)
-                        std::stable_sort(chunk.begin(), chunk.end(), [&](int a, int b2) { return (a % ti_n) < (b2 % ti_n); });
-                    for (int pass = 0; pass < 2; ++pass)
-                        for (int t2 : chunk) {
-                            const int ti = t2 % ti_n, tj = t2 / ti_n;
-                            const bool border = (ti == 0 || ti == ti_n - 1 || tj == 0 || tj == tj_n - 1);
-                            if (env_mode == 3 ? (pass == 0) : (border == (pass == 0))) h[(size_t)(o++) * 8 + x] = t2;
-                        }
-                }
-                SBTV_HIP(ctx, hipStreamSynchronize(ctx->stream));
-                SBTV_HIP(ctx, hipMemcpy(od, h.data(), sizeof(int) * nt, hipMemcpyHostToDevice));
+    static const bool order_off = [] {
+        const char *e = getenv("SBTV_TILE_ORDER");
+        return e && e[0] == '0';
+    }();
+    auto order_table = [&](int cj, int ti_n, int tj_n, const int **out) -> int {
+        *out = nullptr;
+        const int nt = ti_n * tj_n;
+        if (order_off || pl->rpl != 2 || nt <= 2 * 256) return 0;
+        int *od = nullptr;
+        const std::string name = "prox.order." + std::to_string(M) + "x" + std::to_string(N) + "." + std::to_string(cj) +
+                                 "." + std::to_string(pl->nw);
+        const bool built = ctx->ws.find(name) != ctx->ws.end();
+        SBTV_TRY(ws_get_t(ctx, name.c_str(), (size_t)nt, &od));
+        if (!built) {
+            std::vector<int> h(nt);
+            const int q8 = nt >> 3, r8 = nt & 7;
+            for (int x = 0; x < 8; ++x) {
+                const int c0 = (x < r8 ? x * (q8 + 1) : r8 * (q8 + 1) + (x - r8) * q8);
+                const int len = q8 + (x < r8 ? 1 : 0);
+                int o = 0;
+                static const int env_mode = [] {
+                    const char *e = getenv("SBTV_TILE_ORDER");
+                    return e ? atoi(e) : 1;
+                }();
+                std::vector<int> chunk;
+                for (int t2 = c0; t2 < c0 + len; ++t2) chunk.push_back(t2);
+                if (env_mode >= 2)
+                    std::stable_sort(chunk.begin(), chunk.end(), [&](int a, int b2) { return (a % ti_n) < (b2 % ti_n); });
+                for (int pass = 0; pass < 2; ++pass)
+                    for (int t2 : chunk) {
+                        const int ti = t2 % ti_n, tj = t2 / ti_n;
+                        const bool border = (ti == 0 || ti == ti_n - 1 || tj == 0 || tj == tj_n - 1);
+                        if (env_mode == 3 ? (pass == 0) : (border == (pass == 0))) h[(size_t)(o++) * 8 + x] = t2;
+                    }
             }
-            pl->order = od;
-        }
+            SBTV_HIP(ctx, hipStreamSynchronize(ctx->stream));
+            SBTV_HIP(ctx, hipMemcpy(od, h.data(), sizeof(int) * nt, hipMemcpyHostToDevice));
+        }
+        *out = od;
+        return 0;
+    };
+    SBTV_TRY(order_table(pl->cj, pl->ftiles_i, pl->ftiles_j, &pl->order));
+    pl->s_cj = pl->cj;
+    pl->s_tiles_i = pl->ftiles_i;
+    pl->s_tiles_j = pl->ftiles_j;
+    pl->s_nblk = pl->fnblk;
+    pl->s_order = pl->order;
+    if (fused_spec_cols() == 5 && fused_esub_wanted() && g_fused.fast && pl->rpl == 2 && pl->cj == 4 && pl->nw == 8 &&
+        pl->minw == 4) {
+        const int core_cols = 5 * pl->nw - FHL - FHJ;
+        pl->s_cj = 5;
+        pl->s_tiles_j = (N + core_cols - 1) / core_cols;
+        pl->s_nblk = pl->s_tiles_i * pl->s_tiles_j;
+        SBTV_TRY(order_table(pl->s_cj, pl->s_tiles_i, pl->s_tiles_j, &pl->s_order));
     }
     SBTV_TRY(ws_get_t(ctx, (t + ".counters").c_str(), (size_t)batch, &pl->counters));
     SBTV_HIP(ctx, hipMemsetAsync(pl->counters, 0, sizeof(unsigned) * batch, ctx->stream));
@@ -786,22 +818,26 @@
         if (g_fused.fast)                                                                                            \
             hipLaunchKernelGGL((chambolle_fused_kernel<CJ_, NW_, MW_, true>), fgrid, dim3(64 * NW_), 0, ctx->stream, \
                                g, pl.pbuf, pl.ctrl, pl.partials, pl.M, pl.N, pl.batch, pl.ftiles_i, pl.fnblk, steps, \
-                               redo, f_out, write_f, pl.counters, kflags, sj, pl.order, FusedStagger{fused_stagger(pl.fnblk)});  \
+                               redo, f_out, write_f, pl.counters, kflags, sj, pl.order, fused_stagger(ctx, pl.fnblk));  \
         else                                                                                                         \
             hipLaunchKernelGGL((chambolle_fused_kernel<CJ_, NW_, MW_, false>), fgrid, dim3(64 * NW_), 0,             \
                                ctx->stream, g, pl.pbuf, pl.ctrl, pl.partials, pl.M, pl.N, pl.batch, pl.ftiles_i,     \
-                               pl.fnblk, steps, redo, f_out, write_f, pl.counters, kflags, sj, pl.order, FusedStagger{fused_stagger(pl.fnblk)}); \
-    }
-            static const bool esub_wanted = [] {
-                const char *e = getenv("SBTV_ERR_SUBSET");
-                return !(e && e[0] == '0');
-            }();
+                               pl.fnblk, steps, redo, f_out, write_f, pl.counters, kflags, sj, pl.order, fused_stagger(ctx, pl.fnblk)); \
+    }
+            const bool esub_wanted = fused_esub_wanted();
+            if (pl.s_cj == 5 && !pl.esub_off && spec == 1 && !redo) {
+                launched = true;
+                fgrid.x = pl.s_nblk + sj.nblocks;
+                hipLaunchKernelGGL((chambolle_fused_kernel<5, 8, 4, true, true>), fgrid, dim3(64 * 8), 0, ctx->stream, g, pl.pbuf,
+                                   pl.ctrl, pl.partials, pl.M, pl.N, pl.batch, pl.s_tiles_i, pl.s_nblk, steps, redo, f_out, write_f,
+                                   pl.counters, kflags, sj, pl.s_order, fused_stagger(ctx, pl.s_nblk));
+            } else
             if (esub_wanted && !pl.esub_off && spec == 1 && !redo && pl.rpl == 2 && pl.cj == 4 && pl.nw == 8 && pl.minw == 4 &&
                 g_fused.fast) {
                 launched = true;
                 hipLaunchKernelGGL((chambolle_fused_kernel<4, 8, 4, true, true>), fgrid, dim3(64 * 8), 0, ctx->stream, g, pl.pbuf,
                                    pl.ctrl, pl.partials, pl.M, pl.N, pl.batch, pl.ftiles_i, pl.fnblk, steps, redo, f_out, write_f,
-                                   pl.counters, kflags, sj, pl.order, FusedStagger{fused_stagger(pl.fnblk)});
+                                   pl.counters, kflags, sj, pl.order, fused_stagger(ctx, pl.fnblk));
             } else
             SBTV_FUSED_CASE(4, 8, 4)
 #undef SBTV_FUSED_CASE
@@ -1000,10 +1036,26 @@
     out[9] = pl.ftiles_i;
     out[10] = pl.ftiles_j;
     out[11] = pl.order != nullptr ? 1 : 0;
-    out[12] = two ? fused_stagger(pl.fnblk) : 0;
+    out[12] = two ? fused_stagger(ctx, pl.fnblk).stagger : 0;
     out[13] = TI;
     out[14] = TJ;
     out[15] = FHJ;
+    return 0;
+}
+
+int sbtv_diag_prox_spec_geometry(sbtv_ctx *ctx, int M, int N, int batch, int out[8]) {
+    if (!ctx || !out || M < 2 || N < 2 || batch < 1) return SBTV_ERR_BADARG;
+    SBTV_HIP(ctx, hipSetDevice(ctx->device));
+    ProxPlan pl;
+    SBTV_TRY(prox_plan(ctx, M, N, batch, &pl));
+    out[0] = pl.s_cj;
+    out[1] = pl.s_cj * pl.nw;
+    out[2] = pl.s_cj * pl.nw - FHL - FHJ;
+    out[3] = pl.s_tiles_i;
+    out[4] = pl.s_tiles_j;
+    out[5] = pl.s_nblk;
+    out[6] = pl.s_order != nullptr ? 1 : 0;
+    out[7] = (pl.rpl == 2) ? fused_stagger(ctx, pl.s_nblk).stagger : 0;
     return 0;
 }
 
diff --git a/semi-blind-image-deblurring-problems-with-tv_amd/csrc/tv_fused.inc b/semi-blind-image-deblurring-problems-with-tv_amd/csrc/tv_fused.inc
--- a/semi-blind-image-deblurring-problems-with-tv_amd/csrc/tv_fused.inc
+++ b/semi-blind-image-deblurring-problems-with-tv_amd/csrc/tv_fused.inc
@@ -390,7 +390,7 @@
     double *pxo = pbuf + (size_t)(dst * 2 + 0) * plane + (size_t)b * P;
     double *pyo = pbuf + (size_t)(dst * 2 + 1) * plane + (size_t)b * P;
     const double *gg = g + (size_t)b * P;
-    __shared__ __attribute__((aligned(16))) double lds[(FRJ + 2 * FNW) * FRI + FH * 64 * FNW];
+    __shared__ __attribute__((aligned(16))) double lds[(FRJ + 2 * FNW) * FRI + FHJ * 64 * FNW];
     int tile;
     {
         const int nt = gridDim.x - nside, bid = blockIdx.x - nside;
@@ -402,7 +402,7 @@
     const int stagger = stg.stagger;
     if (stagger > 0) {
         const int bid = blockIdx.x - nside;
-        if (bid >= 256 && bid < 512 && b == 0)
+        if (bid >= stg.lo && bid < stg.hi && b == 0)
             for (int q = 0; q < stagger; ++q) __builtin_amdgcn_s_sleep(18);
     }
     const int ti = tile % tiles_i, tj = tile / tiles_i;
diff --git a/semi-blind-image-deblurring-problems-with-tv_amd/sbtv/_lib.py b/semi-blind-image-deblurring-problems-with-tv_amd/sbtv/_lib.py
--- a/semi-blind-image-deblurring-problems-with-tv_amd/sbtv/_lib.py
+++ b/semi-blind-image-deblurring-problems-with-tv_amd/sbtv/_lib.py
@@ -178,6 +178,7 @@
     "sbtv_diag_canary": (_I, [_P, _I, C.POINTER(_I), C.POINTER(_I), C.POINTER(_I)]),
     "sbtv_diag_prox_variant": (_I, [_P, _I, _I, _I, C.POINTER(_I)]),
     "sbtv_diag_prox_geometry": (_I, [_P, _I, _I, _I, C.POINTER(_I)]),
+    "sbtv_diag_prox_spec_geometry": (_I, [_P, _I, _I, _I, C.POINTER(_I)]),
     "sbtv_diag_fft_plan": (_I, [_P, _I, _I, _I, C.POINTER(_I)]),
     "sbtv_diag_spectral_pass": (_I, [_P, C.POINTER(sbtv_diag_pass)]),
     "sbtv_last_host_stats": (_I, [_P, C.POINTER(_D)]),
@@ -296,6 +297,13 @@
         out = (_I * 16)()
         self.check(self.lib.sbtv_diag_prox_geometry(self.h, int(M), int(N), int(batch), out))
         g = dict(zip(self.GEOMETRY, out))
+        g["order"] = bool(g["order"])
+        return g
+
+    def prox_spec_geometry(self, M, N, batch=1):
+        out = (_I * 8)()
+        self.check(self.lib.sbtv_diag_prox_spec_geometry(self.h, int(M), int(N), int(batch), out))
+        g = dict(zip(("cols_per_wave", "region_cols", "core_cols", "tiles_i", "tiles_j", "tiles", "order", "stagger"), out))
         g["order"] = bool(g["order"])
         return g
 
diff --git a/semi-blind-image-deblurring-problems-with-tv_amd/sbtv/salsa.py b/semi-blind-image-deblurring-problems-with-tv_amd/sbtv/salsa.py
--- a/semi-blind-image-deblurring-problems-with-tv_amd/sbtv/salsa.py
+++ b/semi-blind-image-deblurring-problems-with-tv_amd/sbtv/salsa.py
@@ -10,7 +10,7 @@
 from .tv import _parse_varargin
 
 _OPTIONS = {"P", "PT", "PSI", "PHI", "TVINITIALIZATION", "TVITERS", "MU", "STOPCRITERION", "TOLERANCEA",
-            "MAXITERA", "INITIALIZATION", "TRUE_X", "AT", "VERBOSE", "LS", "SEED", "SPECULATE"}
+            "MAXITERA", "INITIALIZATION", "TRUE_X", "AT", "VERBOSE", "LS", "SEED", "SPECULATE", "CHAMBOLLETOL"}
 
 
 def SALSA_v2(y, A, tau, *varargin, ctx=None, **kw):
@@ -61,6 +61,7 @@
     so.TViters = int(opts.get("TVITERS", 5))
     so.tolA = float(opts.get("TOLERANCEA", 0.001))
     so.speculate = int(opts.get("SPECULATE", so.speculate))
+    so.chambolle_tol = float(opts.get("CHAMBOLLETOL", so.chambolle_tol))
     yi = L.Images(y)
     B, M, N = yi.B, yi.M, yi.N
     init = opts.get("INITIALIZATION", 0)
```
